# ronghanghu/vit_10b_fsdp_example

Hardware: AMD Instinct MI355X
Metric: images/sec (whole node) for ViT-10B bs=128 224px --fake_data (higher is better)
Workload: dtype bf16; 1 GPU; model=ViT-10B (5120d/32h/32L, patch14, 224px), global_batch=128, seq_len=256, parallelism=fsdp1, grad_ckpt=True, grad_ckpt_blocks=13, fuse_residual=False, init=device

## Files before the change

### csrc/bindings.cpp

```cpp

#include <torch/extension.h>

std::vector<torch::Tensor> layernorm_fwd(torch::Tensor x, torch::Tensor w,
                                         torch::Tensor b, double eps);
std::vector<torch::Tensor> layernorm_bwd(torch::Tensor dy, torch::Tensor x,
                                         torch::Tensor w, torch::Tensor mean,
                                         torch::Tensor rstd);
std::vector<torch::Tensor> layernorm_add_fwd(torch::Tensor x,
                                             torch::Tensor res,
                                             torch::Tensor w, torch::Tensor b,
                                             double eps);
std::vector<torch::Tensor> layernorm_add_bwd(torch::Tensor dy,
                                             torch::Tensor dsum,
                                             torch::Tensor sum,
                                             torch::Tensor w,
                                             torch::Tensor mean,
                                             torch::Tensor rstd);

void fused_adamw(std::vector<torch::Tensor> params,
                 std::vector<torch::Tensor> grads,
                 std::vector<torch::Tensor> exp_avgs,
                 std::vector<torch::Tensor> exp_avg_sqs,
                 std::vector<c10::optional<torch::Tensor>> mirrors,
                 double lr,
                 double beta1, double beta2, double eps, double weight_decay,
                 double bias_c1, double bias_c2,
                 c10::optional<torch::Tensor> grad_scale,
                 double grad_prescale);
torch::Tensor multi_tensor_sqnorm(std::vector<torch::Tensor> tensors);
void multi_tensor_scale(std::vector<torch::Tensor> tensors, double factor);
void multi_tensor_scale_tensor(std::vector<torch::Tensor> tensors,
                               torch::Tensor factor);

std::vector<torch::Tensor> cross_entropy_fwd(torch::Tensor logits,
                                             torch::Tensor target);
torch::Tensor cross_entropy_bwd(torch::Tensor dloss, torch::Tensor logits,
                                torch::Tensor target, torch::Tensor lse);

std::vector<torch::Tensor> fmha_fwd(torch::Tensor q, torch::Tensor k,
                                    torch::Tensor v, double scale,
                                    double p_drop, long seed);
std::vector<torch::Tensor> fmha_bwd(torch::Tensor dout, torch::Tensor q,
                                    torch::Tensor k, torch::Tensor v,
                                    torch::Tensor o, torch::Tensor lse,
                                    double scale, double p_drop, long seed);
std::vector<torch::Tensor> fmha_fwd_qkv(torch::Tensor qkv, long num_heads,
                                        double scale, double p_drop,
                                        long seed);
torch::Tensor fmha_bwd_qkv(torch::Tensor dout, torch::Tensor qkv,
                           torch::Tensor o, torch::Tensor lse,
                           long num_heads, double scale, double p_drop,
                           long seed);
torch::Tensor fmha_rowdot(torch::Tensor dout, torch::Tensor o);
std::vector<torch::Tensor> gelu_bwd_colsum(torch::Tensor dy, torch::Tensor x);
std::vector<torch::Tensor> gelu_bwd_colsum_t(torch::Tensor dy,
                                             torch::Tensor x);
std::vector<torch::Tensor> gelu_dropout_bwd_colsum(torch::Tensor dy,
                                                   torch::Tensor x, double p,
                                                   long seed);
std::vector<torch::Tensor> gelu_dropout_bwd_colsum_t(torch::Tensor dy,
                                                     torch::Tensor x, double p,
                                                     long seed);
torch::Tensor transpose2d(torch::Tensor x);
std::vector<torch::Tensor> transpose_colsum(torch::Tensor x);
torch::Tensor dropout_fwd(torch::Tensor x, double p, long seed);
torch::Tensor dropout_add_fwd(torch::Tensor x, torch::Tensor res, double p,
                              long seed);
torch::Tensor gelu_dropout_fwd(torch::Tensor x, double p, long seed);
torch::Tensor gelu_dropout_bwd(torch::Tensor dy, torch::Tensor x, double p,
                               long seed);
torch::Tensor mfma_probe(torch::Tensor a, torch::Tensor b);
torch::Tensor mfma32_probe(torch::Tensor a, torch::Tensor b);
torch::Tensor tr16_probe(long mode);
std::vector<torch::Tensor> wgrad_gemm(torch::Tensor a, torch::Tensor b,
                                      bool with_bias);
torch::Tensor fwd_gemm(torch::Tensor x, torch::Tensor w,
                       c10::optional<torch::Tensor> bias);
std::vector<torch::Tensor> fwd_gemm_gelu(torch::Tensor x, torch::Tensor w,
                                         torch::Tensor bias);
torch::Tensor lt_gemm(torch::Tensor a, torch::Tensor b, long algo_index,
                      c10::optional<torch::Tensor> bias);
std::vector<torch::Tensor> lt_gemm_gelu(torch::Tensor a, torch::Tensor b,
                                        c10::optional<torch::Tensor> bias,
                                        long algo_index);
std::vector<torch::Tensor> lt_gemm_dgelu_bgrad(torch::Tensor dy,
                                               torch::Tensor w,
                                               torch::Tensor aux,
                                               long algo_index);
torch::Tensor dgrad_tn(torch::Tensor dy, torch::Tensor w, long algo_index);

PYBIND11_MODULE(TORCH_EXTENSION_NAME, m) {
  m.doc() = "MI355X-native CDNA4 kernels for the FSDP ViT framework";
  m.def("layernorm_fwd", &layernorm_fwd, "LayerNorm forward (bf16, fp32 stats)");
  m.def("layernorm_bwd", &layernorm_bwd, "LayerNorm backward");
  m.def("layernorm_add_fwd", &layernorm_add_fwd,
        "fused residual-add + LayerNorm forward");
  m.def("layernorm_add_bwd", &layernorm_add_bwd,
        "fused residual-add + LayerNorm backward");
  m.def("fused_adamw", &fused_adamw,
        "multi-tensor AdamW step (fp32 master, fp32/bf16 grads with "
        "folded prescale + deferred clip)",
        py::arg("params"), py::arg("grads"), py::arg("exp_avgs"),
        py::arg("exp_avg_sqs"), py::arg("mirrors"), py::arg("lr"),
        py::arg("beta1"), py::arg("beta2"), py::arg("eps"),
        py::arg("weight_decay"), py::arg("bias_c1"), py::arg("bias_c2"),
        py::arg("grad_scale") = py::none(), py::arg("grad_prescale") = 1.0);
  m.def("multi_tensor_sqnorm", &multi_tensor_sqnorm,
        "sum of squares over tensor list");
  m.def("multi_tensor_scale", &multi_tensor_scale, "in-place scalar scale");
  m.def("multi_tensor_scale_tensor", &multi_tensor_scale_tensor,
        "in-place scale by device scalar");
  m.def("cross_entropy_fwd", &cross_entropy_fwd, "fused softmax CE forward");
  m.def("cross_entropy_bwd", &cross_entropy_bwd, "fused softmax CE backward");
  m.def("fmha_fwd", &fmha_fwd,
        "flash attention forward (bf16, head_dim<=192; in-kernel "
        "attention dropout via a counter-hash mask)",
        py::arg("q"), py::arg("k"), py::arg("v"), py::arg("scale"),
        py::arg("p_drop") = 0.0, py::arg("seed") = 0);
  m.def("fmha_bwd", &fmha_bwd,
        "flash attention backward (fused FA2-style; regenerates the "
        "dropout mask from the seed)",
        py::arg("dout"), py::arg("q"), py::arg("k"), py::arg("v"),
        py::arg("o"), py::arg("lse"), py::arg("scale"),
        py::arg("p_drop") = 0.0, py::arg("seed") = 0);
  m.def("fmha_fwd_qkv", &fmha_fwd_qkv,
        "flash attention forward on the fused [B,T,3,H,D] qkv projection "
        "(zero-copy strided IO, O returned as [B,T,E])",
        py::arg("qkv"), py::arg("num_heads"), py::arg("scale"),
        py::arg("p_drop") = 0.0, py::arg("seed") = 0);
  m.def("fmha_bwd_qkv", &fmha_bwd_qkv,
        "flash attention backward producing the fused dqkv [B,T,3,H,D]",
        py::arg("dout"), py::arg("qkv"), py::arg("o"), py::arg("lse"),
        py::arg("num_heads"), py::arg("scale"), py::arg("p_drop") = 0.0,
        py::arg("seed") = 0);
  m.def("fmha_rowdot", &fmha_rowdot,
        "Delta = rowsum(dO * O) of the attention backward, fp32 [B,H,T], "
        "for contiguous [B,H,T,D] operands",
        py::arg("dout"), py::arg("o"));
  m.def("gelu_bwd_colsum", &gelu_bwd_colsum,
        "(dx, colsum): exact-erf GELU backward and the bf16 column sums "
        "of dx over all rows (fc1 bias gradient) in one pass",
        py::arg("dy"), py::arg("x"));
  m.def("gelu_bwd_colsum_t", &gelu_bwd_colsum_t,
        "(dx, colsum, dx^T): gelu_bwd_colsum with dx^T [hid, rows] as a "
        "third output; dx and colsum are bit-identical to gelu_bwd_colsum's",
        py::arg("dy"), py::arg("x"));
  m.def("transpose2d", &transpose2d,
        "bf16 [R, C] contiguous -> [C, R] contiguous (C % 8 == 0)",
        py::arg("x"));
  m.def("transpose_colsum", &transpose_colsum,
        "(x^T, colsum): transpose2d plus the bf16 column sums of x over "
        "all rows (a linear's bias gradient) from the same read; fp32 "
        "accumulation in a fixed order",
        py::arg("x"));
  m.def("dropout_fwd", &dropout_fwd,
        "hidden dropout with the in-kernel (seed, row, col) hash mask: "
        "keep ? x / (1 - p) : 0; the same call on dy is its backward",
        py::arg("x"), py::arg("p"), py::arg("seed"));
  m.def("dropout_add_fwd", &dropout_add_fwd,
        "x + dropout(res) in one pass (residual add with the branch's "
        "dropout folded in), rounded once",
        py::arg("x"), py::arg("res"), py::arg("p"), py::arg("seed"));
  m.def("gelu_dropout_fwd", &gelu_dropout_fwd,
        "dropout(gelu(x)) in one pass, exact-erf GELU, rounded once",
        py::arg("x"), py::arg("p"), py::arg("seed"));
  m.def("gelu_dropout_bwd", &gelu_dropout_bwd,
        "backward of gelu_dropout_fwd from dy and the pre-activation x; "
        "regenerates the mask from the seed",
        py::arg("dy"), py::arg("x"), py::arg("p"), py::arg("seed"));
  m.def("gelu_dropout_bwd_colsum", &gelu_dropout_bwd_colsum,
        "(dx, colsum): gelu_dropout_bwd and the bf16 column sums of dx "
        "over all rows (fc1 bias gradient) in one pass; dx is "
        "bit-identical to gelu_dropout_bwd's",
        py::arg("dy"), py::arg("x"), py::arg("p"), py::arg("seed"));
  m.def("gelu_dropout_bwd_colsum_t", &gelu_dropout_bwd_colsum_t,
        "(dx, colsum, dx^T): gelu_dropout_bwd_colsum with dx^T [hid, rows] "
        "as a third output; dx and colsum are bit-identical to "
        "gelu_dropout_bwd_colsum's",
        py::arg("dy"), py::arg("x"), py::arg("p"), py::arg("seed"));
  m.def("mfma_probe", &mfma_probe, "16x16x32 bf16 MFMA layout probe");
  m.def("mfma32_probe", &mfma32_probe, "32x32x16 bf16 MFMA layout probe");
  m.def("tr16_probe", &tr16_probe, "ds_read_b64_tr_b16 semantics probe");
  m.def("wgrad_gemm", &wgrad_gemm,
        "C = A^T B weight-gradient GEMM (bf16, tr16 transpose reads)");
  m.def("fwd_gemm", &fwd_gemm,
        "C = X W^T forward Linear GEMM (+fused bias), hand-written CDNA4 "
        "MFMA (csrc/fgemm.hip)",
        py::arg("x"), py::arg("w"), py::arg("bias") = py::none());
  m.def("fwd_gemm_gelu", &fwd_gemm_gelu,
        "(gelu(X W^T + bias), pre-activation) with the EXACT erf GELU "
        "fused into the hand-written forward GEMM epilogue",
        py::arg("x"), py::arg("w"), py::arg("bias"));
  m.def("lt_gemm", &lt_gemm,
        "row-major bf16 GEMM (+optional fused bias epilogue) via "
        "hipblaslt-ext with an explicit algorithm index (-1 = library "
        "heuristic); offline-search apply path, see "
        "csrc/tools/hipblaslt_search.cpp",
        py::arg("a"), py::arg("b"), py::arg("algo_index") = -1,
        py::arg("bias") = py::none());
  m.def("lt_gemm_gelu", &lt_gemm_gelu,
        "(gelu(a@b+bias), pre-activation aux) in one hipblaslt-ext GEMM "
        "(GELU_AUX epilogue; tanh-approx GELU)",
        py::arg("a"), py::arg("b"), py::arg("bias") = py::none(),
        py::arg("algo_index") = -1);
  m.def("lt_gemm_dgelu_bgrad", &lt_gemm_dgelu_bgrad,
        "(dgelu(dy@w, aux), column-sum bias grad) in one hipblaslt-ext "
        "GEMM (DGELU_BGRAD epilogue)",
        py::arg("dy"), py::arg("w"), py::arg("aux"),
        py::arg("algo_index") = -1);
  m.def("dgrad_tn", &dgrad_tn,
        "dx [tok, in] = dy [tok, out] @ w [out, in] as the library's TN "
        "GEMM on w^T, which csrc/transpose.hip writes into a scratch "
        "buffer on every call; row-contiguous bf16 operands, in and out "
        "multiples of 8, w 16-byte aligned",
        py::arg("dy"), py::arg("w"), py::arg("algo_index") = -1);
}
```

### csrc/fmha.hip

```cpp

#ifndef VITFSDP_KERNELS_ONLY
#include <ATen/cuda/CUDAContext.h>
#include <torch/extension.h>

#include <cstdlib>
#include <cstring>
#include <type_traits>
#endif

#include "mfma_tiles.h"

namespace {

constexpr int kBlockThreads = 256;
constexpr int kKTile = 32;
constexpr int kMaxD = 192;

template <int D>
struct FmhaShapes {
  static constexpr int QSub = (D <= 96) ? 2 : 1;
  static constexpr int QTile = 64 * QSub;
  static constexpr int DP = ((D + 31) / 32) * 32;
  static constexpr int NKC = DP / 32;
  static constexpr int NC = D / 16;
  static constexpr int KStride = DP + 8;
  static constexpr int PStride = kKTile + 8;
  static constexpr int VRow = D + 16;
  struct Shared {
    short k_tile[2][kKTile][KStride];
    short v_tile[2][kKTile][VRow];
  };
  struct SharedDQ {
    short k_tile[kKTile][KStride];
    short v_tile[kKTile][KStride];
  };
  struct SharedDKV {
    short q_tile[32][KStride];
    short do_tile[32][KStride];
    short pt_tile[4][16][PStride];
    short dst_tile[4][16][PStride];
  };
};


struct QkvStrides {
  long qb, qh, qt;
  long ob, oh, ot;
};


template <int D, bool DROP = false>
__global__ __launch_bounds__(kBlockThreads, 3) void fmha_fwd_kernel(
    const short* __restrict__ q, const short* __restrict__ k,
    const short* __restrict__ v, short* __restrict__ o,
    float* __restrict__ lse_out, int T, int H, QkvStrides st, float scale,
    unsigned drop_thresh = 0, float drop_rscale = 1.f, unsigned seed = 0) {
  using S = FmhaShapes<D>;
  constexpr int DP = S::DP, NKC = S::NKC, NC = S::NC;
  constexpr int kQSub = S::QSub;
  constexpr int kQTile = S::QTile;
  HIP_DYNAMIC_SHARED(char, smem_raw)
  typename S::Shared& sm = *reinterpret_cast<typename S::Shared*>(smem_raw);

  const int lane = threadIdx.x & 63;
  const int wave = threadIdx.x >> 6;
  const int col = lane & 15;
  const int seg = lane >> 4;
  const long bh = blockIdx.x;
  const int q_base = blockIdx.y * kQTile;
  const int q_row0 = q_base + wave * (16 * kQSub);

  const int b_idx = (int)(bh / H), h_idx = (int)(bh % H);
  const long qkv_off = (long)b_idx * st.qb + (long)h_idx * st.qh;
  const long o_off = (long)b_idx * st.ob + (long)h_idx * st.oh;

  using KStage = TileStage<kKTile, DP, D, kBlockThreads>;
  using VStage = TileStage<kKTile, D, D, kBlockThreads>;
  const KStage k_stg;
  const VStage v_stg;

  bf16x8 q_frag[kQSub][NKC];
#pragma unroll
  for (int qs = 0; qs < kQSub; ++qs) {
    const int q_row = q_row0 + 16 * qs + col;
    load_row_frags<NKC, D>(q + qkv_off + (long)q_row * st.qt, q_row < T, seg,
                           q_frag[qs]);
  }

  float m_run[kQSub], l_run[kQSub];
  f32x4 o_acc[kQSub][NC];
#pragma unroll
  for (int qs = 0; qs < kQSub; ++qs) {
    m_run[qs] = -INFINITY;
    l_run[qs] = 0.f;
#pragma unroll
    for (int c = 0; c < NC; ++c) o_acc[qs][c] = f32x4{0.f, 0.f, 0.f, 0.f};
  }

  bf16x8 stage[KStage::N > VStage::N ? KStage::N : VStage::N];
  auto issue_k_loads = [&](int k_base) {
    k_stg.load(k + qkv_off, st.qt, k_base, T, stage);
  };
  auto write_k_tile = [&](int buf) { k_stg.store(sm.k_tile[buf], stage); };
  auto issue_v_loads = [&](int k_base) {
    v_stg.load(v + qkv_off, st.qt, k_base, T, stage);
  };
  auto write_v_tile = [&](int buf) { v_stg.store(sm.v_tile[buf], stage); };

  const int n_ktiles = (T + kKTile - 1) / kKTile;
  issue_k_loads(0);
  write_k_tile(0);
  issue_v_loads(0);
  write_v_tile(0);
  __syncthreads();

  int cur = 0;
  for (int kt = 0; kt < n_ktiles; ++kt) {
    const int k_base = kt * kKTile;
    const bool has_next = kt + 1 < n_ktiles;

    if (has_next) issue_k_loads(k_base + kKTile);

#pragma unroll
    for (int qs = 0; qs < kQSub; ++qs) {
      f32x4 st_frag[2] = {{0.f, 0.f, 0.f, 0.f}, {0.f, 0.f, 0.f, 0.f}};
#pragma unroll
      for (int kk = 0; kk < 2; ++kk) {
#pragma unroll
        for (int kc = 0; kc < NKC; ++kc) {
          bf16x8 a_frag = *reinterpret_cast<const bf16x8*>(
              &sm.k_tile[cur][kk * 16 + col][kc * 32 + seg * 8]);
          st_frag[kk] = __builtin_amdgcn_mfma_f32_16x16x32_bf16(
              a_frag, q_frag[qs][kc], st_frag[kk], 0, 0, 0);
        }
      }

      float sc[2][4];
      float my_max = -INFINITY;
#pragma unroll
      for (int kk = 0; kk < 2; ++kk) {
#pragma unroll
        for (int r = 0; r < 4; ++r) {
          float sv = st_frag[kk][r] * scale;
          if (k_base + 16 * kk + seg * 4 + r >= T) sv = -INFINITY;
          sc[kk][r] = sv;
          my_max = fmaxf(my_max, sv);
        }
      }
      my_max = fmaxf(my_max, __shfl_xor(my_max, 16));
      my_max = fmaxf(my_max, __shfl_xor(my_max, 32));
      const float m_new = fmaxf(m_run[qs], my_max);
      const float alpha = __expf(m_run[qs] - m_new);
      m_run[qs] = m_new;

      float p[2][4];
      float row_sum = 0.f;
#pragma unroll
      for (int kk = 0; kk < 2; ++kk) {
#pragma unroll
        for (int r = 0; r < 4; ++r) {
          const float pv =
              (sc[kk][r] == -INFINITY) ? 0.f : __expf(sc[kk][r] - m_new);
          p[kk][r] = pv;
          row_sum += pv;
        }
      }
      row_sum += __shfl_xor(row_sum, 16);
      row_sum += __shfl_xor(row_sum, 32);
      l_run[qs] = l_run[qs] * alpha + row_sum;

      if (DROP) {
        const unsigned qg = (unsigned)(bh * T + q_row0 + 16 * qs + col);
#pragma unroll
        for (int kk = 0; kk < 2; ++kk) {
#pragma unroll
          for (int r = 0; r < 4; ++r) {
            const unsigned kg = (unsigned)(k_base + 16 * kk + seg * 4 + r);
            p[kk][r] = dropout_hash(seed, qg, kg) >= drop_thresh
                           ? p[kk][r] * drop_rscale
                           : 0.f;
          }
        }
      }

      unsigned pk[2][2];
#pragma unroll
      for (int kk = 0; kk < 2; ++kk) {
#pragma unroll
        for (int rr = 0; rr < 2; ++rr)
          pk[kk][rr] = pack_bf16x2(p[kk][2 * rr], p[kk][2 * rr + 1]);
      }
      const bf16x8 pa = c_to_a_layout(pk, seg, col);

#pragma unroll
      for (int r = 0; r < 4; ++r) {
        const float alpha_o = __shfl(alpha, seg * 4 + r);
#pragma unroll
        for (int c = 0; c < NC; ++c) o_acc[qs][c][r] *= alpha_o;
      }

      if (qs == kQSub - 1 && has_next) {
        write_k_tile(cur ^ 1);
        issue_v_loads(k_base + kKTile);
      }

      const unsigned v_lds_base =
          (unsigned)__builtin_amdgcn_groupstaticsize() +
          (unsigned)(offsetof(typename S::Shared, v_tile)) +
          (unsigned)cur * (unsigned)sizeof(sm.v_tile[0]);
      mfma_tr_ring<NC, S::VRow>(pa, v_lds_base, seg, col, o_acc[qs]);
    }

    if (has_next) write_v_tile(cur ^ 1);
    __syncthreads();
    cur ^= 1;
  }

#pragma unroll
  for (int qs = 0; qs < kQSub; ++qs) {
    if (seg == 0) {
      const int q_row = q_row0 + 16 * qs + col;
      if (q_row < T) {
        lse_out[bh * T + q_row] = m_run[qs] + __logf(l_run[qs]);
      }
    }
#pragma unroll
    for (int r = 0; r < 4; ++r) {
      const float l_row = __shfl(l_run[qs], seg * 4 + r);
      const int q_row = q_row0 + 16 * qs + seg * 4 + r;
      if (q_row >= T) continue;
      const float inv_l = (l_row > 0.f) ? 1.f / l_row : 0.f;
      const long out_base = o_off + (long)q_row * st.ot;
#pragma unroll
      for (int c = 0; c < NC; ++c) {
        o[out_base + c * 16 + col] =
            (short)f32_to_bf16(o_acc[qs][c][r] * inv_l);
      }
    }
  }
}

template <int D, bool DROP = false>
__global__ __launch_bounds__(kBlockThreads, 3) void fmha_bwd_dq_kernel(
    const short* __restrict__ q, const short* __restrict__ k,
    const short* __restrict__ v, const short* __restrict__ dout,
    const float* __restrict__ lse, const float* __restrict__ delta,
    short* __restrict__ dq, int T, int H, QkvStrides st, float scale,
    unsigned drop_thresh = 0, float drop_rscale = 1.f, unsigned seed = 0) {
  using S = FmhaShapes<D>;
  constexpr int DP = S::DP, NKC = S::NKC, NC = S::NC;
  constexpr int kQSub = S::QSub;
  constexpr int kQTile = S::QTile;
  HIP_DYNAMIC_SHARED(char, smem_raw)
  typename S::SharedDQ& sm =
      *reinterpret_cast<typename S::SharedDQ*>(smem_raw);

  const int lane = threadIdx.x & 63;
  const int wave = threadIdx.x >> 6;
  const int col = lane & 15;
  const int seg = lane >> 4;
  const long bh = blockIdx.x;
  const int q_base = blockIdx.y * kQTile;
  const int q_row0 = q_base + wave * (16 * kQSub);
  const int b_idx = (int)(bh / H), h_idx = (int)(bh % H);
  const long qkv_off = (long)b_idx * st.qb + (long)h_idx * st.qh;
  const long o_off = (long)b_idx * st.ob + (long)h_idx * st.oh;

  bf16x8 q_frag[kQSub][NKC], do_frag[kQSub][NKC];
  float lse_q[kQSub], delta_q[kQSub];
#pragma unroll
  for (int qs = 0; qs < kQSub; ++qs) {
    const int q_row = q_row0 + 16 * qs + col;
    const bool valid = q_row < T;
    load_row_frags<NKC, D>(q + qkv_off + (long)q_row * st.qt, valid, seg,
                           q_frag[qs]);
    load_row_frags<NKC, D>(dout + o_off + (long)q_row * st.ot, valid, seg,
                           do_frag[qs]);
    lse_q[qs] = valid ? lse[bh * T + q_row] : 0.f;
    delta_q[qs] = valid ? delta[bh * T + q_row] : 0.f;
  }

  f32x4 dq_acc[kQSub][NC];
#pragma unroll
  for (int qs = 0; qs < kQSub; ++qs)
#pragma unroll
    for (int c = 0; c < NC; ++c) dq_acc[qs][c] = f32x4{0.f, 0.f, 0.f, 0.f};

  using Stage = TileStage<kKTile, DP, D, kBlockThreads>;
  const Stage stg;
  bf16x8 kst[Stage::N], vst[Stage::N];
  auto issue_kv_loads = [&](int k_base) {
    stg.load(k + qkv_off, st.qt, k_base, T, kst);
    stg.load(v + qkv_off, st.qt, k_base, T, vst);
  };
  auto write_kv_tiles = [&]() {
    stg.store(sm.k_tile, kst);
    stg.store(sm.v_tile, vst);
  };

  const int n_ktiles = (T + kKTile - 1) / kKTile;
  issue_kv_loads(0);
  write_kv_tiles();
  __syncthreads();
  for (int kt = 0; kt < n_ktiles; ++kt) {
    const int k_base = kt * kKTile;
    const bool has_next = kt + 1 < n_ktiles;
    if (has_next) issue_kv_loads(k_base + kKTile);

#pragma unroll
    for (int qs = 0; qs < kQSub; ++qs) {
      f32x4 st_frag[2] = {{0.f, 0.f, 0.f, 0.f}, {0.f, 0.f, 0.f, 0.f}};
      f32x4 dpt_frag[2] = {{0.f, 0.f, 0.f, 0.f}, {0.f, 0.f, 0.f, 0.f}};
#pragma unroll
      for (int kk = 0; kk < 2; ++kk) {
#pragma unroll
        for (int kc = 0; kc < NKC; ++kc) {
          bf16x8 kb = *reinterpret_cast<const bf16x8*>(
              &sm.k_tile[kk * 16 + col][kc * 32 + seg * 8]);
          bf16x8 vb = *reinterpret_cast<const bf16x8*>(
              &sm.v_tile[kk * 16 + col][kc * 32 + seg * 8]);
          st_frag[kk] = __builtin_amdgcn_mfma_f32_16x16x32_bf16(
              kb, q_frag[qs][kc], st_frag[kk], 0, 0, 0);
          dpt_frag[kk] = __builtin_amdgcn_mfma_f32_16x16x32_bf16(
              vb, do_frag[qs][kc], dpt_frag[kk], 0, 0, 0);
        }
      }

      unsigned pk[2][2];
#pragma unroll
      for (int kk = 0; kk < 2; ++kk) {
#pragma unroll
        for (int rr = 0; rr < 2; ++rr) {
          float ds[2] = {0.f, 0.f};
#pragma unroll
          for (int h = 0; h < 2; ++h) {
            const int r = 2 * rr + h;
            const int k_idx = k_base + 16 * kk + seg * 4 + r;
            if (k_idx < T) {
              const float pv =
                  __expf(st_frag[kk][r] * scale - lse_q[qs]);
              float dp = dpt_frag[kk][r];
              if (DROP) {
                const unsigned qg = (unsigned)(bh * T + q_row0 + 16 * qs + col);
                dp = dropout_hash(seed, qg, (unsigned)k_idx) >= drop_thresh
                         ? dp * drop_rscale
                         : 0.f;
              }
              ds[h] = scale * pv * (dp - delta_q[qs]);
            }
          }
          pk[kk][rr] = pack_bf16x2(ds[0], ds[1]);
        }
      }
      const bf16x8 ds_frag = c_to_a_layout(pk, seg, col);

      const unsigned k_lds_base =
          (unsigned)__builtin_amdgcn_groupstaticsize() +
          (unsigned)offsetof(typename S::SharedDQ, k_tile);
      mfma_tr_ring<NC, S::KStride>(ds_frag, k_lds_base, seg, col,
                                   dq_acc[qs]);
    }

    if (has_next) {
      __syncthreads();
      write_kv_tiles();
      __syncthreads();
    }
  }

#pragma unroll
  for (int qs = 0; qs < kQSub; ++qs) {
#pragma unroll
    for (int r = 0; r < 4; ++r) {
      const int q_row = q_row0 + 16 * qs + seg * 4 + r;
      if (q_row >= T) continue;
      const long out_base = qkv_off + (long)q_row * st.qt;
#pragma unroll
      for (int c = 0; c < NC; ++c) {
        dq[out_base + c * 16 + col] = (short)f32_to_bf16(dq_acc[qs][c][r]);
      }
    }
  }
}

template <int D, bool DROP = false>
__global__ __launch_bounds__(kBlockThreads, 2) void fmha_bwd_dkv_kernel(
    const short* __restrict__ q, const short* __restrict__ k,
    const short* __restrict__ v, const short* __restrict__ dout,
    const float* __restrict__ lse, const float* __restrict__ delta,
    short* __restrict__ dk, short* __restrict__ dv, int T, int H,
    QkvStrides st, float scale,
    unsigned drop_thresh = 0, float drop_rscale = 1.f, unsigned seed = 0) {
  using S = FmhaShapes<D>;
  constexpr int DP = S::DP, NKC = S::NKC, NC = S::NC;
  constexpr int kQStream = 32;
  HIP_DYNAMIC_SHARED(char, smem_raw)
  typename S::SharedDKV& sm =
      *reinterpret_cast<typename S::SharedDKV*>(smem_raw);

  const int lane = threadIdx.x & 63;
  const int wave = threadIdx.x >> 6;
  const int col = lane & 15;
  const int seg = lane >> 4;
  const long bh = blockIdx.x;
  const int k_base = blockIdx.y * 64;
  const int k_row0 = k_base + wave * 16;
  const int b_idx = (int)(bh / H), h_idx = (int)(bh % H);
  const long qkv_off = (long)b_idx * st.qb + (long)h_idx * st.qh;
  const long o_off = (long)b_idx * st.ob + (long)h_idx * st.oh;

  bf16x8 k_frag[NKC], v_frag[NKC];
  {
    const int k_row = k_row0 + col;
    const long base = qkv_off + (long)k_row * st.qt;
    load_row_frags<NKC, D>(k + base, k_row < T, seg, k_frag);
    load_row_frags<NKC, D>(v + base, k_row < T, seg, v_frag);
  }

  f32x4 dk_acc[NC], dv_acc[NC];
#pragma unroll
  for (int c = 0; c < NC; ++c) {
    dk_acc[c] = f32x4{0.f, 0.f, 0.f, 0.f};
    dv_acc[c] = f32x4{0.f, 0.f, 0.f, 0.f};
  }

  using Stage = TileStage<kQStream, DP, D, kBlockThreads>;
  const Stage stg;
  bf16x8 q_st[Stage::N], do_st[Stage::N];
  auto issue_qdo_loads = [&](int q_base) {
    stg.load(q + qkv_off, st.qt, q_base, T, q_st);
    stg.load(dout + o_off, st.ot, q_base, T, do_st);
  };
  auto write_qdo_tiles = [&]() {
    stg.store(sm.q_tile, q_st);
    stg.store(sm.do_tile, do_st);
  };

  const int n_qtiles = (T + kQStream - 1) / kQStream;
  issue_qdo_loads(0);
  write_qdo_tiles();
  __syncthreads();
  for (int qt = 0; qt < n_qtiles; ++qt) {
    const int q_base = qt * kQStream;
    const bool has_next = qt + 1 < n_qtiles;
    if (has_next) issue_qdo_loads(q_base + kQStream);

    f32x4 st_frag[2] = {{0.f, 0.f, 0.f, 0.f}, {0.f, 0.f, 0.f, 0.f}};
    f32x4 dpt_frag[2] = {{0.f, 0.f, 0.f, 0.f}, {0.f, 0.f, 0.f, 0.f}};
#pragma unroll
    for (int qq = 0; qq < 2; ++qq) {
#pragma unroll
      for (int kc = 0; kc < NKC; ++kc) {
        bf16x8 qb = *reinterpret_cast<const bf16x8*>(
            &sm.q_tile[qq * 16 + col][kc * 32 + seg * 8]);
        bf16x8 dob = *reinterpret_cast<const bf16x8*>(
            &sm.do_tile[qq * 16 + col][kc * 32 + seg * 8]);
        st_frag[qq] = __builtin_amdgcn_mfma_f32_16x16x32_bf16(
            k_frag[kc], qb, st_frag[qq], 0, 0, 0);
        dpt_frag[qq] = __builtin_amdgcn_mfma_f32_16x16x32_bf16(
            v_frag[kc], dob, dpt_frag[qq], 0, 0, 0);
      }
    }

#pragma unroll
    for (int qq = 0; qq < 2; ++qq) {
      const int q_idx = q_base + qq * 16 + col;
      const bool q_ok = q_idx < T;
      const float l = q_ok ? lse[bh * T + q_idx] : 0.f;
      const float dlt = q_ok ? delta[bh * T + q_idx] : 0.f;
#pragma unroll
      for (int r = 0; r < 4; ++r) {
        float pt = 0.f, dst = 0.f;
        if (q_ok) {
          pt = __expf(st_frag[qq][r] * scale - l);
          float dp = dpt_frag[qq][r];
          if (DROP) {
            const unsigned qg = (unsigned)(bh * T + q_idx);
            const unsigned kg = (unsigned)(k_row0 + seg * 4 + r);
            const bool keep = dropout_hash(seed, qg, kg) >= drop_thresh;
            dp = keep ? dp * drop_rscale : 0.f;
            dst = scale * pt * (dp - dlt);
            pt = keep ? pt * drop_rscale : 0.f;
          } else {
            dst = scale * pt * (dp - dlt);
          }
        }
        sm.pt_tile[wave][seg * 4 + r][qq * 16 + col] =
            (short)f32_to_bf16(pt);
        sm.dst_tile[wave][seg * 4 + r][qq * 16 + col] =
            (short)f32_to_bf16(dst);
      }
    }
    asm volatile("s_waitcnt lgkmcnt(0)" ::: "memory");

    bf16x8 pt_frag = *reinterpret_cast<const bf16x8*>(
        &sm.pt_tile[wave][col][seg * 8]);
    bf16x8 dst_frag = *reinterpret_cast<const bf16x8*>(
        &sm.dst_tile[wave][col][seg * 8]);
    const unsigned base0 = (unsigned)__builtin_amdgcn_groupstaticsize();
    const unsigned q_lds_base =
        base0 + (unsigned)offsetof(typename S::SharedDKV, q_tile);
    const unsigned do_lds_base =
        base0 + (unsigned)offsetof(typename S::SharedDKV, do_tile);
    mfma_tr_ring<NC, S::KStride>(pt_frag, do_lds_base, seg, col, dv_acc);
    mfma_tr_ring<NC, S::KStride>(dst_frag, q_lds_base, seg, col, dk_acc);
    if (has_next) {
      __syncthreads();
      write_qdo_tiles();
      __syncthreads();
    }
  }

#pragma unroll
  for (int r = 0; r < 4; ++r) {
    const int k_row = k_row0 + seg * 4 + r;
    if (k_row >= T) continue;
    const long out_base = qkv_off + (long)k_row * st.qt;
#pragma unroll
    for (int c = 0; c < NC; ++c) {
      dk[out_base + c * 16 + col] = (short)f32_to_bf16(dk_acc[c][r]);
      dv[out_base + c * 16 + col] = (short)f32_to_bf16(dv_acc[c][r]);
    }
  }
}

constexpr int kRowdotLanes = 8;
constexpr int kRowdotRows = kBlockThreads / kRowdotLanes;
constexpr int kRowdotMaxLoads = kMaxD / 8 / kRowdotLanes;

__global__ __launch_bounds__(kBlockThreads) void fmha_rowdot_kernel(
    const ushort8_t* __restrict__ dout, const ushort8_t* __restrict__ o,
    float* __restrict__ delta, int n_rows, int T, int H, int nvec,
    long sob, long soh, long sot ,
    int h_fast) {
  const int g = threadIdx.x % kRowdotLanes;
  const int slot = threadIdx.x / kRowdotLanes;
  for (long r0 = (long)blockIdx.x * kRowdotRows; r0 < n_rows;
       r0 += (long)gridDim.x * kRowdotRows) {
    const bool ok = r0 + slot < n_rows;
    const unsigned r = ok ? (unsigned)(r0 + slot) : 0u;
    unsigned b, h, t;
    if (h_fast) {
      h = r % (unsigned)H;
      t = (r / (unsigned)H) % (unsigned)T;
    } else {
      t = r % (unsigned)T;
      h = (r / (unsigned)T) % (unsigned)H;
    }
    b = r / ((unsigned)T * (unsigned)H);
    const long base = (long)b * sob + (long)h * soh + (long)t * sot;

    ushort8_t dv[kRowdotMaxLoads], ov[kRowdotMaxLoads];
#pragma unroll
    for (int k = 0; k < kRowdotMaxLoads; ++k) {
      const int v = g + k * kRowdotLanes;
      if (ok && v < nvec) {
        dv[k] = dout[base + v];
        ov[k] = o[base + v];
      }
    }
    float acc[8];
#pragma unroll
    for (int j = 0; j < 8; ++j) acc[j] = 0.f;
#pragma unroll
    for (int k = 0; k < kRowdotMaxLoads; ++k) {
      const int v = g + k * kRowdotLanes;
      if (ok && v < nvec) {
#pragma unroll
        for (int j = 0; j < 8; ++j)
          acc[j] += bf16_to_f32(dv[k][j]) * bf16_to_f32(ov[k][j]);
      }
    }
#pragma unroll
    for (int off = kRowdotLanes / 2; off > 0; off >>= 1) {
#pragma unroll
      for (int j = 0; j < 8; ++j) acc[j] += __shfl_xor(acc[j], off);
    }
#pragma unroll
    for (int j = 0; j < 4; ++j) acc[j] += acc[j + 4];
    acc[0] += acc[2];
    acc[1] += acc[3];
    acc[0] += acc[1];
    if (ok && g == 0) delta[((long)b * H + h) * T + t] = acc[0];
  }
}

__global__ __launch_bounds__(64) void fmha_rowdot_scalar_kernel(
    const unsigned short* __restrict__ dout,
    const unsigned short* __restrict__ o, float* __restrict__ delta, int T,
    int H, int D, long sob, long soh, long sot) {
  const long row = blockIdx.x;
  const int t = (int)(row % T);
  const int h = (int)((row / T) % H);
  const long b = row / ((long)T * H);
  const long base = b * sob + (long)h * soh + (long)t * sot;
  float acc = 0.f;
  for (int i = threadIdx.x; i < D; i += 64)
    acc += bf16_to_f32(dout[base + i]) * bf16_to_f32(o[base + i]);
  acc = wave_all_sum(acc);
  if (threadIdx.x == 0) delta[row] = acc;
}

__global__ __launch_bounds__(256) void fmha_dsoftmax_kernel(
    const unsigned short* __restrict__ s_raw,
    const unsigned short* __restrict__ dp, const float* __restrict__ lse,
    const float* __restrict__ delta, unsigned short* __restrict__ p_out,
    unsigned short* __restrict__ ds_out, int T, float scale) {
  const long row = blockIdx.x;
  const float row_lse = lse[row];
  const float row_delta = delta[row];
  const long base = row * T;
  if ((T & 7) == 0) {
    const int nvec = T / 8;
    const ushort8_t* sv = (const ushort8_t*)(s_raw + base);
    const ushort8_t* dpv = (const ushort8_t*)(dp + base);
    ushort8_t* pv = (ushort8_t*)(p_out + base);
    ushort8_t* dsv = (ushort8_t*)(ds_out + base);
    for (int i = threadIdx.x; i < nvec; i += 256) {
      ushort8_t s8 = sv[i], d8 = dpv[i], p8, ds8;
#pragma unroll
      for (int j = 0; j < 8; ++j) {
        const float p = __expf(bf16_to_f32(s8[j]) * scale - row_lse);
        p8[j] = f32_to_bf16(p);
        ds8[j] = f32_to_bf16(scale * p * (bf16_to_f32(d8[j]) - row_delta));
      }
      pv[i] = p8;
      dsv[i] = ds8;
    }
  } else {
    for (int i = threadIdx.x; i < T; i += 256) {
      const float p = __expf(bf16_to_f32(s_raw[base + i]) * scale - row_lse);
      p_out[base + i] = f32_to_bf16(p);
      ds_out[base + i] =
          f32_to_bf16(scale * p * (bf16_to_f32(dp[base + i]) - row_delta));
    }
  }
}

#ifdef VITFSDP_KERNELS_ONLY
template __global__ void fmha_fwd_kernel<160, false>(
    const short*, const short*, const short*, short*, float*, int, int,
    QkvStrides, float, unsigned, float, unsigned);
template __global__ void fmha_fwd_kernel<160, true>(
    const short*, const short*, const short*, short*, float*, int, int,
    QkvStrides, float, unsigned, float, unsigned);
template __global__ void fmha_fwd_kernel<64, false>(
    const short*, const short*, const short*, short*, float*, int, int,
    QkvStrides, float, unsigned, float, unsigned);
#define VITFSDP_INSTANTIATE_BWD(D_, DROP_)                                  \
  template __global__ void fmha_bwd_dq_kernel<D_, DROP_>(                    \
      const short*, const short*, const short*, const short*, const float*,  \
      const float*, short*, int, int, QkvStrides, float, unsigned, float,    \
      unsigned);                                                             \
  template __global__ void fmha_bwd_dkv_kernel<D_, DROP_>(                   \
      const short*, const short*, const short*, const short*, const float*,  \
      const float*, short*, short*, int, int, QkvStrides, float, unsigned,   \
      float, unsigned);
VITFSDP_INSTANTIATE_BWD(160, false)
VITFSDP_INSTANTIATE_BWD(160, true)
VITFSDP_INSTANTIATE_BWD(64, false)
#undef VITFSDP_INSTANTIATE_BWD
#else
struct FmhaArgs {
  const short *q, *k, *v;
  short* o;
  int B, H, T;
  QkvStrides st;
  float scale;
  float p_drop = 0.f;
  unsigned seed = 0;
};

inline unsigned drop_threshold(float p) {
  if (p <= 0.f) return 0u;
  double t = (double)p * 4294967296.0;
  return t >= 4294967295.0 ? 4294967295u : (unsigned)t;
}

template <typename F>
void with_dropout(const FmhaArgs& a, F&& f) {
  if (a.p_drop > 0.f) {
    f(std::true_type{}, drop_threshold(a.p_drop), 1.f / (1.f - a.p_drop),
      a.seed);
  } else {
    f(std::false_type{}, 0u, 1.f, 0u);
  }
}

template <int D>
void launch_fmha_fwd(const FmhaArgs& a, torch::Tensor& lse) {
  dim3 grid((unsigned)((long)a.B * a.H),
            (a.T + FmhaShapes<D>::QTile - 1) / FmhaShapes<D>::QTile);
  auto stream = at::cuda::getCurrentCUDAStream();
  with_dropout(a, [&](auto drop, unsigned thr, float rs, unsigned seed) {
    hipLaunchKernelGGL((fmha_fwd_kernel<D, decltype(drop)::value>), grid,
                       dim3(kBlockThreads),
                       sizeof(typename FmhaShapes<D>::Shared), stream, a.q,
                       a.k, a.v, a.o, lse.data_ptr<float>(), a.T, a.H, a.st,
                       a.scale, thr, rs, seed);
  });
  HIP_CHECK_LAST();
}

template <int D>
void launch_fmha_bwd(const FmhaArgs& a, const torch::Tensor& lse,
                     const torch::Tensor& delta, short* dq, short* dk,
                     short* dv) {
  using S = FmhaShapes<D>;
  auto stream = at::cuda::getCurrentCUDAStream();
  const unsigned BH = (unsigned)((long)a.B * a.H);
  dim3 grid_dq(BH, (a.T + S::QTile - 1) / S::QTile);
  dim3 grid_dkv(BH, (a.T + 63) / 64);
  with_dropout(a, [&](auto drop, unsigned thr, float rs, unsigned seed) {
    constexpr bool kDrop = decltype(drop)::value;
    hipLaunchKernelGGL((fmha_bwd_dq_kernel<D, kDrop>), grid_dq,
                       dim3(kBlockThreads), sizeof(typename S::SharedDQ),
                       stream, a.q, a.k, a.v, a.o ,
                       lse.data_ptr<float>(), delta.data_ptr<float>(), dq,
                       a.T, a.H, a.st, a.scale, thr, rs, seed);
    HIP_CHECK_LAST();
    hipLaunchKernelGGL((fmha_bwd_dkv_kernel<D, kDrop>), grid_dkv,
                       dim3(kBlockThreads), sizeof(typename S::SharedDKV),
                       stream, a.q, a.k, a.v, a.o ,
                       lse.data_ptr<float>(), delta.data_ptr<float>(), dk, dv,
                       a.T, a.H, a.st, a.scale, thr, rs, seed);
    HIP_CHECK_LAST();
  });
}

#define VITFSDP_FMHA_DISPATCH(D_, expr)                               \
  switch (D_) {                                                       \
    case 16: { constexpr int kD = 16; expr; break; }                  \
    case 32: { constexpr int kD = 32; expr; break; }                  \
    case 48: { constexpr int kD = 48; expr; break; }                  \
    case 64: { constexpr int kD = 64; expr; break; }                  \
    case 80: { constexpr int kD = 80; expr; break; }                  \
    case 96: { constexpr int kD = 96; expr; break; }                  \
    case 112: { constexpr int kD = 112; expr; break; }                \
    case 128: { constexpr int kD = 128; expr; break; }                \
    case 144: { constexpr int kD = 144; expr; break; }                \
    case 160: { constexpr int kD = 160; expr; break; }                \
    case 176: { constexpr int kD = 176; expr; break; }                \
    case 192: { constexpr int kD = 192; expr; break; }                \
    default: TORCH_CHECK(false, "fmha: unsupported head_dim ", D_);   \
  }

#endif

}

#ifndef VITFSDP_KERNELS_ONLY
namespace {

QkvStrides contiguous_strides(int H, int T, int D) {
  QkvStrides st;
  st.qh = (long)T * D;
  st.qb = (long)H * st.qh;
  st.qt = D;
  st.ob = st.qb;
  st.oh = st.qh;
  st.ot = st.qt;
  return st;
}

QkvStrides fused_qkv_strides(int T, int H, int D) {
  QkvStrides st;
  st.qt = 3L * H * D;
  st.qb = (long)T * st.qt;
  st.qh = D;
  st.ot = (long)H * D;
  st.ob = (long)T * st.ot;
  st.oh = D;
  return st;
}

torch::Tensor run_rowdot(const torch::Tensor& dout, const torch::Tensor& o,
                         int B, int H, int T, int D, const QkvStrides& st) {
  auto delta = torch::empty({B, H, T}, dout.options().dtype(torch::kFloat32));
  auto stream = at::cuda::getCurrentCUDAStream();
  const long n_rows = (long)B * H * T;
  if (n_rows == 0) return delta;
  const bool aligned =
      ((reinterpret_cast<uintptr_t>(dout.data_ptr()) |
        reinterpret_cast<uintptr_t>(o.data_ptr())) & 15) == 0 &&
      D % 8 == 0 && D <= kMaxD && st.ob % 8 == 0 && st.oh % 8 == 0 &&
      st.ot % 8 == 0;
  if (aligned && n_rows < (1L << 31)) {
    const long n_blocks =
        std::min<long>((n_rows + kRowdotRows - 1) / kRowdotRows, 2048);
    hipLaunchKernelGGL(fmha_rowdot_kernel, dim3((unsigned)n_blocks),
                       dim3(kBlockThreads), 0, stream,
                       (const ushort8_t*)dout.data_ptr(),
                       (const ushort8_t*)o.data_ptr(), delta.data_ptr<float>(),
                       (int)n_rows, T, H, D / 8, st.ob / 8, st.oh / 8,
                       st.ot / 8, st.oh < st.ot ? 1 : 0);
  } else {
    hipLaunchKernelGGL(fmha_rowdot_scalar_kernel, dim3(n_rows), dim3(64), 0,
                       stream, (const unsigned short*)dout.data_ptr(),
                       (const unsigned short*)o.data_ptr(),
                       delta.data_ptr<float>(), T, H, D, st.ob, st.oh, st.ot);
  }
  HIP_CHECK_LAST();
  return delta;
}

bool supported_head_dim(long D) { return D >= 16 && D <= kMaxD && D % 16 == 0; }

void check_bwd_operand(const char* fn, const char* name,
                       const torch::Tensor& t, const torch::Tensor& like,
                       at::IntArrayRef shape) {
  TORCH_CHECK(t.is_cuda() && t.device() == like.device(), fn, ": ", name,
              " must be a GPU tensor on the device of the other operands");
  TORCH_CHECK(t.scalar_type() == torch::kBFloat16, fn, ": ", name,
              " must be bf16, got ", t.scalar_type());
  TORCH_CHECK(t.sizes() == shape, fn, ": ", name, " must have shape ", shape,
              ", got ", t.sizes());
  TORCH_CHECK(t.is_contiguous(), fn, ": ", name, " must be contiguous");
}

void check_bwd_lse(const char* fn, const torch::Tensor& lse,
                   const torch::Tensor& like, long B, long H, long T) {
  TORCH_CHECK(lse.is_cuda() && lse.device() == like.device(), fn,
              ": lse must be a GPU tensor on the device of the other operands");
  TORCH_CHECK(lse.scalar_type() == torch::kFloat32, fn,
              ": lse must be fp32, got ", lse.scalar_type());
  TORCH_CHECK(lse.dim() == 3 && lse.size(0) == B && lse.size(1) == H &&
                  lse.size(2) == T,
              fn, ": lse must have shape [B, H, T] = [", B, ", ", H, ", ", T,
              "], got ", lse.sizes());
  TORCH_CHECK(lse.is_contiguous(), fn, ": lse must be contiguous");
}

}


std::vector<torch::Tensor> fmha_fwd(torch::Tensor q, torch::Tensor k,
                                    torch::Tensor v, double scale,
                                    double p_drop, long seed) {
  TORCH_CHECK(q.is_cuda() && q.is_contiguous() && k.is_contiguous() &&
              v.is_contiguous());
  TORCH_CHECK(q.scalar_type() == torch::kBFloat16, "fmha_fwd: bf16 only");
  TORCH_CHECK(q.dim() == 4, "fmha_fwd: [B, H, T, D]");
  const int B = q.size(0), H = q.size(1), T = q.size(2), D = q.size(3);
  TORCH_CHECK(D % 16 == 0 && D <= kMaxD,
              "fmha_fwd: head_dim must be a multiple of 16 and <= ", kMaxD);

  auto o = torch::empty_like(q);
  auto lse = torch::empty({B, H, T}, q.options().dtype(torch::kFloat32));
  FmhaArgs a{(const short*)q.data_ptr(), (const short*)k.data_ptr(),
             (const short*)v.data_ptr(), (short*)o.data_ptr(),
             B, H, T, contiguous_strides(H, T, D), (float)scale,
             (float)p_drop, (unsigned)seed};
  VITFSDP_FMHA_DISPATCH(D, launch_fmha_fwd<kD>(a, lse));
  return {o, lse};
}

std::vector<torch::Tensor> fmha_bwd(torch::Tensor dout, torch::Tensor q,
                                    torch::Tensor k, torch::Tensor v,
                                    torch::Tensor o, torch::Tensor lse,
                                    double scale, double p_drop, long seed) {
  TORCH_CHECK(q.is_cuda() && q.dim() == 4,
              "fmha_bwd: q must be a GPU tensor [B, H, T, D]");
  TORCH_CHECK(supported_head_dim(q.size(3)),
              "fmha_bwd: head_dim must be a multiple of 16 and <= ", kMaxD,
              ", got ", q.size(3));
  check_bwd_operand("fmha_bwd", "q", q, q, q.sizes());
  check_bwd_operand("fmha_bwd", "k", k, q, q.sizes());
  check_bwd_operand("fmha_bwd", "v", v, q, q.sizes());
  check_bwd_operand("fmha_bwd", "o", o, q, q.sizes());
  check_bwd_operand("fmha_bwd", "dout", dout, q, q.sizes());
  check_bwd_lse("fmha_bwd", lse, q, q.size(0), q.size(1), q.size(2));
  const int B = q.size(0), H = q.size(1), T = q.size(2), D = q.size(3);
  const QkvStrides st = contiguous_strides(H, T, D);
  auto delta = run_rowdot(dout, o, B, H, T, D, st);
  auto stream = at::cuda::getCurrentCUDAStream();

  static const bool use_compose = [] {
    const char* e = getenv("VITFSDP_FMHA_BWD");
    return e != nullptr && strcmp(e, "compose") == 0;
  }();
  if (use_compose) {
    auto s_raw = at::matmul(q, k.transpose(-2, -1));
    auto dp = at::matmul(dout, v.transpose(-2, -1));
    auto p = torch::empty_like(s_raw);
    auto ds = torch::empty_like(s_raw);
    hipLaunchKernelGGL(fmha_dsoftmax_kernel, dim3((long)B * H * T), dim3(256),
                       0, stream, (const unsigned short*)s_raw.data_ptr(),
                       (const unsigned short*)dp.data_ptr(),
                       lse.data_ptr<float>(), delta.data_ptr<float>(),
                       (unsigned short*)p.data_ptr(),
                       (unsigned short*)ds.data_ptr(), T, (float)scale);
    HIP_CHECK_LAST();
    auto dv = at::matmul(p.transpose(-2, -1), dout);
    auto dq = at::matmul(ds, k);
    auto dk = at::matmul(ds.transpose(-2, -1), q);
    return {dq, dk, dv};
  }

  auto dq = torch::empty_like(q);
  auto dk = torch::empty_like(k);
  auto dv = torch::empty_like(v);
  FmhaArgs a{(const short*)q.data_ptr(), (const short*)k.data_ptr(),
             (const short*)v.data_ptr(), (short*)dout.data_ptr(),
             B, H, T, st, (float)scale, (float)p_drop, (unsigned)seed};
  VITFSDP_FMHA_DISPATCH(
      D, launch_fmha_bwd<kD>(a, lse, delta, (short*)dq.data_ptr(),
                             (short*)dk.data_ptr(), (short*)dv.data_ptr()));
  return {dq, dk, dv};
}

torch::Tensor fmha_rowdot(torch::Tensor dout, torch::Tensor o) {
  TORCH_CHECK(dout.is_cuda() && o.is_cuda() && dout.is_contiguous() &&
                  o.is_contiguous(),
              "fmha_rowdot: contiguous GPU tensors");
  TORCH_CHECK(dout.scalar_type() == torch::kBFloat16 &&
                  o.scalar_type() == torch::kBFloat16,
              "fmha_rowdot: bf16 only");
  TORCH_CHECK(dout.dim() == 4 && dout.sizes() == o.sizes(),
              "fmha_rowdot: two [B, H, T, D] tensors of one shape");
  const int B = dout.size(0), H = dout.size(1), T = dout.size(2),
            D = dout.size(3);
  TORCH_CHECK(D % 16 == 0 && D <= kMaxD,
              "fmha_rowdot: head_dim must be a multiple of 16 and <= ", kMaxD);
  return run_rowdot(dout, o, B, H, T, D, contiguous_strides(H, T, D));
}


std::vector<torch::Tensor> fmha_fwd_qkv(torch::Tensor qkv, long num_heads,
                                        double scale, double p_drop,
                                        long seed) {
  TORCH_CHECK(qkv.is_cuda() && qkv.is_contiguous() && qkv.dim() == 5 &&
                  qkv.size(2) == 3 && qkv.size(3) == num_heads,
              "fmha_fwd_qkv: expected contiguous [B, T, 3, H, D]");
  TORCH_CHECK(qkv.scalar_type() == torch::kBFloat16, "fmha: bf16 only");
  const int B = qkv.size(0), T = qkv.size(1), H = qkv.size(3),
            D = qkv.size(4);
  TORCH_CHECK(D % 16 == 0 && D <= kMaxD,
              "fmha: head_dim must be a multiple of 16 and <= ", kMaxD);
  const QkvStrides st = fused_qkv_strides(T, H, D);

  auto o = torch::empty({B, T, (long)H * D}, qkv.options());
  auto lse = torch::empty({B, H, T}, qkv.options().dtype(torch::kFloat32));
  const short* base = (const short*)qkv.data_ptr();
  FmhaArgs a{base, base + (long)H * D, base + 2L * H * D,
             (short*)o.data_ptr(), B, H, T, st, (float)scale,
             (float)p_drop, (unsigned)seed};
  VITFSDP_FMHA_DISPATCH(D, launch_fmha_fwd<kD>(a, lse));
  return {o, lse};
}

torch::Tensor fmha_bwd_qkv(torch::Tensor dout, torch::Tensor qkv,
                           torch::Tensor o, torch::Tensor lse,
                           long num_heads, double scale, double p_drop,
                           long seed) {
  TORCH_CHECK(qkv.is_cuda() && qkv.is_contiguous() && qkv.dim() == 5 &&
                  qkv.size(2) == 3 && qkv.size(3) == num_heads,
              "fmha_bwd_qkv: expected contiguous GPU qkv [B, T, 3, H, D]");
  TORCH_CHECK(qkv.scalar_type() == torch::kBFloat16,
              "fmha_bwd_qkv: qkv must be bf16, got ", qkv.scalar_type());
  TORCH_CHECK(supported_head_dim(qkv.size(4)),
              "fmha_bwd_qkv: head_dim must be a multiple of 16 and <= ", kMaxD,
              ", got ", qkv.size(4));
  {
    const long b = qkv.size(0), t = qkv.size(1), h = qkv.size(3),
               d = qkv.size(4);
    const std::vector<long> flat{b, t, h * d}, split{b, t, h, d};
    check_bwd_operand("fmha_bwd_qkv", "o", o, qkv,
                      o.dim() == 4 ? split : flat);
    check_bwd_operand("fmha_bwd_qkv", "dout", dout, qkv,
                      dout.dim() == 4 ? split : flat);
    check_bwd_lse("fmha_bwd_qkv", lse, qkv, b, h, t);
  }
  const int B = qkv.size(0), T = qkv.size(1), H = qkv.size(3),
            D = qkv.size(4);
  const QkvStrides st = fused_qkv_strides(T, H, D);
  auto delta = run_rowdot(dout, o, B, H, T, D, st);

  auto dqkv = torch::empty_like(qkv);
  const short* base = (const short*)qkv.data_ptr();
  short* dbase = (short*)dqkv.data_ptr();
  FmhaArgs a{base, base + (long)H * D, base + 2L * H * D,
             (short*)dout.data_ptr(), B, H, T, st, (float)scale,
             (float)p_drop, (unsigned)seed};
  VITFSDP_FMHA_DISPATCH(
      D, launch_fmha_bwd<kD>(a, lse, delta, dbase, dbase + (long)H * D,
                             dbase + 2L * H * D));
  return dqkv;
}
#endif
```

### csrc/mfma_tiles.h

```cpp
#pragma once

#include "common.h"

typedef __attribute__((ext_vector_type(8))) short bf16x8;
typedef __attribute__((ext_vector_type(4))) float f32x4;
typedef __attribute__((ext_vector_type(16))) float f32x16;
typedef __attribute__((ext_vector_type(2))) unsigned int u32x2;


__device__ __forceinline__ u32x2 tr16_read(unsigned lds_byte_addr) {
  u32x2 v;
  asm volatile("ds_read_b64_tr_b16 %0, %1 offset:0"
               : "=v"(v)
               : "v"(lds_byte_addr));
  return v;
}

template <int OFF>
__device__ __forceinline__ u32x2 tr16_read_at(unsigned lds_byte_addr) {
  static_assert(OFF >= 0 && OFF < 65536, "ds offset field is 16 bits");
  u32x2 v;
  asm volatile("ds_read_b64_tr_b16 %0, %1 offset:%2"
               : "=v"(v)
               : "v"(lds_byte_addr), "n"(OFF));
  return v;
}

template <int N>
__device__ __forceinline__ void lds_wait(u32x2& lo, u32x2& hi) {
  asm volatile("s_waitcnt lgkmcnt(%[cnt])"
               : "+v"(lo), "+v"(hi)
               : [cnt] "i"(N)
               : "memory");
}

__device__ __forceinline__ bf16x8 frag_from(u32x2 lo, u32x2 hi) {
  union {
    u32x2 uu[2];
    bf16x8 v;
  } cv;
  cv.uu[0] = lo;
  cv.uu[1] = hi;
  return cv.v;
}

__device__ __forceinline__ unsigned pack_bf16x2(float lo, float hi) {
  return (unsigned)f32_to_bf16(lo) | ((unsigned)f32_to_bf16(hi) << 16);
}

template <int NC, int STRIDE>
__device__ __forceinline__ void mfma_tr_ring(bf16x8 a, unsigned lds_base,
                                             int seg, int col,
                                             f32x4 (&acc)[NC]) {
  const unsigned lane_base =
      lds_base +
      2u * (unsigned)((seg * 8 + (col >> 2)) * STRIDE + (col & 3) * 4);
  u32x2 bf[2][2];
#pragma unroll
  for (int h = 0; h < 2; ++h)
    bf[0][h] = tr16_read(lane_base + 2u * (4 * h * STRIDE));
#pragma unroll
  for (int c = 0; c < NC; ++c) {
    const int cur = c & 1;
    if (c + 1 < NC) {
#pragma unroll
      for (int h = 0; h < 2; ++h)
        bf[cur ^ 1][h] =
            tr16_read(lane_base + 2u * (4 * h * STRIDE + (c + 1) * 16));
      lds_wait<2>(bf[cur][0], bf[cur][1]);
    } else {
      lds_wait<0>(bf[cur][0], bf[cur][1]);
    }
    acc[c] = __builtin_amdgcn_mfma_f32_16x16x32_bf16(
        a, frag_from(bf[cur][0], bf[cur][1]), acc[c], 0, 0, 0);
  }
}

__device__ __forceinline__ bf16x8 c_to_a_layout(const unsigned (&pk)[2][2],
                                                int seg, int col) {
  union {
    unsigned u[4];
    bf16x8 v;
  } cvt;
#pragma unroll
  for (int j2 = 0; j2 < 4; ++j2) {
    const int src = col + 16 * ((seg & 1) * 2 + (j2 >> 1));
    const unsigned lo = (unsigned)__shfl((int)pk[0][j2 & 1], src);
    const unsigned hi = (unsigned)__shfl((int)pk[1][j2 & 1], src);
    cvt.u[j2] = (seg >> 1) ? hi : lo;
  }
  return cvt.v;
}

template <int NKC, int D>
__device__ __forceinline__ void load_row_frags(const short* __restrict__ p,
                                               bool valid, int seg,
                                               bf16x8 (&frag)[NKC]) {
#pragma unroll
  for (int kc = 0; kc < NKC; ++kc) {
    const int d0 = kc * 32 + seg * 8;
    if (valid && d0 + 8 <= D) {
      frag[kc] = *reinterpret_cast<const bf16x8*>(&p[d0]);
    } else {
#pragma unroll
      for (int j = 0; j < 8; ++j)
        frag[kc][j] = (valid && d0 + j < D) ? p[d0 + j] : (short)0;
    }
  }
}

template <int ROWS, int COLS, int D, int THREADS>
struct TileStage {
  static constexpr int VPR = COLS / 8;
  static constexpr int N = (ROWS * VPR + THREADS - 1) / THREADS;
  int r[N], c[N];
  __device__ __forceinline__ TileStage() {
#pragma unroll
    for (int i = 0; i < N; ++i) {
      const int idx = (int)threadIdx.x + i * THREADS;
      r[i] = idx / VPR;
      c[i] = (idx % VPR) * 8;
    }
  }
  template <int M>
  __device__ __forceinline__ void load(const short* __restrict__ p,
                                       long row_stride, int row0, int T,
                                       bf16x8 (&st)[M]) const {
#pragma unroll
    for (int i = 0; i < N; ++i) {
      bf16x8 val = {0, 0, 0, 0, 0, 0, 0, 0};
      const int row = row0 + r[i];
      if (r[i] < ROWS && row < T && (COLS <= D || c[i] < D)) {
        val = *reinterpret_cast<const bf16x8*>(
            &p[(long)row * row_stride + c[i]]);
      }
      st[i] = val;
    }
  }
  template <int STRIDE, int M>
  __device__ __forceinline__ void store(short (*tile)[STRIDE],
                                        const bf16x8 (&st)[M]) const {
#pragma unroll
    for (int i = 0; i < N; ++i) {
      if (r[i] < ROWS) {
        *reinterpret_cast<bf16x8*>(&tile[r[i]][c[i]]) = st[i];
      }
    }
  }
};

__device__ __forceinline__ int xcd_swizzle_m_major(int bid, int nwg) {
  return (bid & 7) * (nwg >> 3) + (bid >> 3);
}

__device__ __forceinline__ void xcd_cluster_tile(int& bx, int& by) {
  bx = blockIdx.x;
  by = blockIdx.y;
  const int gx = gridDim.x, gy = gridDim.y;
  const int nwg = gx * gy;
  const int bid = (int)(blockIdx.x + blockIdx.y * gx);
  int sx = 2, sy = 4;
  if (gy % 4 != 0) {
    if (gy % 2 == 0) { sx = 4; sy = 2; }
    else { sx = 8; sy = 1; }
  }
  if ((nwg & 7) == 0 && gx % sx == 0 && gy % sy == 0) {
    const int xcd = bid & 7, cid = bid >> 3;
    const int lw = gx / sx, lh = gy / sy;
    const int gm = (lw % 4 == 0) ? 4 : ((lw % 2 == 0) ? 2 : 1);
    const int per_band = gm * lh;
    const int band = cid / per_band, r = cid % per_band;
    bx = (xcd % sx) * lw + band * gm + (r % gm);
    by = (xcd / sx) * lh + r / gm;
  } else if ((nwg & 7) == 0) {
    const int swz = xcd_swizzle_m_major(bid, nwg);
    bx = swz % gx;
    by = swz / gx;
  }
}
```

### csrc/probes.hip

```cpp

#ifndef VITFSDP_KERNELS_ONLY
#include <ATen/cuda/CUDAContext.h>
#include <torch/extension.h>
#endif

#include "mfma_tiles.h"

namespace {

__global__ __launch_bounds__(64) void tr16_probe_kernel(
    unsigned short* __restrict__ out, int mode) {
  HIP_DYNAMIC_SHARED(char, smem_raw)
  unsigned short* lds = reinterpret_cast<unsigned short*>(smem_raw);
  for (int i = threadIdx.x; i < 1024; i += 64) lds[i] = (unsigned short)i;
  __syncthreads();
  const int lane = threadIdx.x & 63;
  unsigned addr_elems;
  switch (mode) {
    case 0: addr_elems = 0; break;
    case 1: addr_elems = (lane & 15) + (lane >> 4) * 64; break;
    case 2: addr_elems = (lane & 15) * 4; break;
    default: addr_elems = lane * 4; break;
  }
  unsigned addr = addr_elems * 2 + (unsigned)__builtin_amdgcn_groupstaticsize();
  u32x2 v = tr16_read(addr);
  asm volatile("s_waitcnt lgkmcnt(0)" : "+v"(v) : : "memory");
  out[lane * 4 + 0] = (unsigned short)(v[0] & 0xffff);
  out[lane * 4 + 1] = (unsigned short)(v[0] >> 16);
  out[lane * 4 + 2] = (unsigned short)(v[1] & 0xffff);
  out[lane * 4 + 3] = (unsigned short)(v[1] >> 16);
}

__global__ __launch_bounds__(64) void mfma32_probe_kernel(
    const float* __restrict__ a, const float* __restrict__ b,
    float* __restrict__ c) {
  const int l = threadIdx.x;
  union { unsigned short u[8]; bf16x8 v; } av, bv;
  for (int j = 0; j < 8; ++j) {
    av.u[j] = f32_to_bf16(a[(l & 31) * 16 + (l >> 5) * 8 + j]);
    bv.u[j] = f32_to_bf16(b[((l >> 5) * 8 + j) * 32 + (l & 31)]);
  }
  f32x16 acc = {};
  acc = __builtin_amdgcn_mfma_f32_32x32x16_bf16(av.v, bv.v, acc, 0, 0, 0);
  for (int g = 0; g < 4; ++g)
    for (int r = 0; r < 4; ++r)
      c[((l >> 5) * 4 + g * 8 + r) * 32 + (l & 31)] = acc[g * 4 + r];
}

__global__ __launch_bounds__(64) void mfma_probe_kernel(
    const float* __restrict__ a, const float* __restrict__ b,
    float* __restrict__ c) {
  const int lane = threadIdx.x & 63;
  const int col = lane & 15, seg = lane >> 4;
  bf16x8 af, bf;
#pragma unroll
  for (int j = 0; j < 8; ++j) {
    af[j] = (short)f32_to_bf16(a[col * 32 + seg * 8 + j]);
    bf[j] = (short)f32_to_bf16(b[(seg * 8 + j) * 16 + col]);
  }
  f32x4 acc = {0.f, 0.f, 0.f, 0.f};
  acc = __builtin_amdgcn_mfma_f32_16x16x32_bf16(af, bf, acc, 0, 0, 0);
#pragma unroll
  for (int r = 0; r < 4; ++r) c[(seg * 4 + r) * 16 + col] = acc[r];
}
}

#ifndef VITFSDP_KERNELS_ONLY
torch::Tensor tr16_probe(long mode) {
  auto out = torch::zeros({64, 4}, torch::TensorOptions()
                                       .dtype(torch::kInt16)
                                       .device(torch::kCUDA));
  auto stream = at::cuda::getCurrentCUDAStream();
  hipLaunchKernelGGL(tr16_probe_kernel, dim3(1), dim3(64), 2048, stream,
                     (unsigned short*)out.data_ptr(), (int)mode);
  HIP_CHECK_LAST();
  return out;
}

torch::Tensor mfma32_probe(torch::Tensor a, torch::Tensor b) {
  TORCH_CHECK(a.is_cuda() && a.is_contiguous() && a.dim() == 2 &&
              a.size(0) == 32 && a.size(1) == 16);
  TORCH_CHECK(b.is_cuda() && b.is_contiguous() && b.dim() == 2 &&
              b.size(0) == 16 && b.size(1) == 32);
  TORCH_CHECK(a.scalar_type() == torch::kFloat32 &&
              b.scalar_type() == torch::kFloat32);
  auto c = torch::zeros({32, 32}, a.options());
  auto stream = at::cuda::getCurrentCUDAStream();
  hipLaunchKernelGGL(mfma32_probe_kernel, dim3(1), dim3(64), 0, stream,
                     a.data_ptr<float>(), b.data_ptr<float>(),
                     c.data_ptr<float>());
  HIP_CHECK_LAST();
  return c;
}

torch::Tensor mfma_probe(torch::Tensor a, torch::Tensor b) {
  TORCH_CHECK(a.is_cuda() && a.sizes() == torch::IntArrayRef({16, 32}));
  TORCH_CHECK(b.is_cuda() && b.sizes() == torch::IntArrayRef({32, 16}));
  auto a32 = a.to(torch::kFloat32).contiguous();
  auto b32 = b.to(torch::kFloat32).contiguous();
  auto c = torch::empty({16, 16}, a32.options());
  auto stream = at::cuda::getCurrentCUDAStream();
  hipLaunchKernelGGL(mfma_probe_kernel, dim3(1), dim3(64), 0, stream,
                     a32.data_ptr<float>(), b32.data_ptr<float>(),
                     c.data_ptr<float>());
  HIP_CHECK_LAST();
  return c;
}
#endif
```

Measured before the change: 70.33 images/sec.

## Add 32-row-tile MFMA 32x32x16 flash attention forward and dQ kernels

Adds new flash-attention forward and dQ-backward kernels built on 32x32x16 bf16 MFMA tiles, with 256 query rows per 512-thread block, double-buffered swizzled LDS staging of K/V, and the accumulator reused directly as the next MFMA operand. For head_dim 160/128 these kernels are routed in by default, replacing the 16-row-tile paths, with env/arg overrides. The aim is higher MFMA throughput and fewer LDS round trips in attention. It raises LDS use (large dynamic shared memory) and lowers occupancy, and attention is a small share of ViT-10B step time.

```diff
diff --git a/csrc/bindings.cpp b/csrc/bindings.cpp
--- a/csrc/bindings.cpp
+++ b/csrc/bindings.cpp
@@ -39,18 +39,19 @@
 
 std::vector<torch::Tensor> fmha_fwd(torch::Tensor q, torch::Tensor k,
                                     torch::Tensor v, double scale,
-                                    double p_drop, long seed);
+                                    double p_drop, long seed, long tile);
 std::vector<torch::Tensor> fmha_bwd(torch::Tensor dout, torch::Tensor q,
                                     torch::Tensor k, torch::Tensor v,
                                     torch::Tensor o, torch::Tensor lse,
-                                    double scale, double p_drop, long seed);
+                                    double scale, double p_drop, long seed,
+                                    long tile);
 std::vector<torch::Tensor> fmha_fwd_qkv(torch::Tensor qkv, long num_heads,
                                         double scale, double p_drop,
-                                        long seed);
+                                        long seed, long tile);
 torch::Tensor fmha_bwd_qkv(torch::Tensor dout, torch::Tensor qkv,
                            torch::Tensor o, torch::Tensor lse,
                            long num_heads, double scale, double p_drop,
-                           long seed);
+                           long seed, long tile);
 torch::Tensor fmha_rowdot(torch::Tensor dout, torch::Tensor o);
 std::vector<torch::Tensor> gelu_bwd_colsum(torch::Tensor dy, torch::Tensor x);
 std::vector<torch::Tensor> gelu_bwd_colsum_t(torch::Tensor dy,
@@ -71,6 +72,8 @@
                                long seed);
 torch::Tensor mfma_probe(torch::Tensor a, torch::Tensor b);
 torch::Tensor mfma32_probe(torch::Tensor a, torch::Tensor b);
+torch::Tensor mfma32_acc_operand_probe(torch::Tensor a0, torch::Tensor b0,
+                                       torch::Tensor a_t);
 torch::Tensor tr16_probe(long mode);
 std::vector<torch::Tensor> wgrad_gemm(torch::Tensor a, torch::Tensor b,
                                       bool with_bias);
@@ -116,23 +119,23 @@
         "flash attention forward (bf16, head_dim<=192; in-kernel "
         "attention dropout via a counter-hash mask)",
         py::arg("q"), py::arg("k"), py::arg("v"), py::arg("scale"),
-        py::arg("p_drop") = 0.0, py::arg("seed") = 0);
+        py::arg("p_drop") = 0.0, py::arg("seed") = 0, py::arg("tile") = 0);
   m.def("fmha_bwd", &fmha_bwd,
         "flash attention backward (fused FA2-style; regenerates the "
         "dropout mask from the seed)",
         py::arg("dout"), py::arg("q"), py::arg("k"), py::arg("v"),
         py::arg("o"), py::arg("lse"), py::arg("scale"),
-        py::arg("p_drop") = 0.0, py::arg("seed") = 0);
+        py::arg("p_drop") = 0.0, py::arg("seed") = 0, py::arg("tile") = 0);
   m.def("fmha_fwd_qkv", &fmha_fwd_qkv,
         "flash attention forward on the fused [B,T,3,H,D] qkv projection "
         "(zero-copy strided IO, O returned as [B,T,E])",
         py::arg("qkv"), py::arg("num_heads"), py::arg("scale"),
-        py::arg("p_drop") = 0.0, py::arg("seed") = 0);
+        py::arg("p_drop") = 0.0, py::arg("seed") = 0, py::arg("tile") = 0);
   m.def("fmha_bwd_qkv", &fmha_bwd_qkv,
         "flash attention backward producing the fused dqkv [B,T,3,H,D]",
         py::arg("dout"), py::arg("qkv"), py::arg("o"), py::arg("lse"),
         py::arg("num_heads"), py::arg("scale"), py::arg("p_drop") = 0.0,
-        py::arg("seed") = 0);
+        py::arg("seed") = 0, py::arg("tile") = 0);
   m.def("fmha_rowdot", &fmha_rowdot,
         "Delta = rowsum(dO * O) of the attention backward, fp32 [B,H,T], "
         "for contiguous [B,H,T,D] operands",
@@ -180,6 +183,10 @@
         py::arg("dy"), py::arg("x"), py::arg("p"), py::arg("seed"));
   m.def("mfma_probe", &mfma_probe, "16x16x32 bf16 MFMA layout probe");
   m.def("mfma32_probe", &mfma32_probe, "32x32x16 bf16 MFMA layout probe");
+  m.def("mfma32_acc_operand_probe", &mfma32_acc_operand_probe,
+        "32x32x16 accumulator tile as the next MFMA's B operand, A by "
+        "permuted transposed LDS reads: returns a_t^T (a0 b0)",
+        py::arg("a0"), py::arg("b0"), py::arg("a_t"));
   m.def("tr16_probe", &tr16_probe, "ds_read_b64_tr_b16 semantics probe");
   m.def("wgrad_gemm", &wgrad_gemm,
         "C = A^T B weight-gradient GEMM (bf16, tr16 transpose reads)");
diff --git a/csrc/fmha.hip b/csrc/fmha.hip
--- a/csrc/fmha.hip
+++ b/csrc/fmha.hip
@@ -9,6 +9,7 @@
 #endif
 
 #include "mfma_tiles.h"
+#include "fmha_tile32.h"
 
 namespace {
 
@@ -43,10 +44,6 @@
 };
 
 
-struct QkvStrides {
-  long qb, qh, qt;
-  long ob, oh, ot;
-};
 
 
 template <int D, bool DROP = false>
@@ -660,6 +657,21 @@
 VITFSDP_INSTANTIATE_BWD(160, true)
 VITFSDP_INSTANTIATE_BWD(64, false)
 #undef VITFSDP_INSTANTIATE_BWD
+#define VITFSDP_INSTANTIATE_T32(D_, DROP_)                                  \
+  template __global__ void fmha_fwd_t32_kernel<D_, DROP_>(                   \
+      const short*, const short*, const short*, short*, float*, int, int,    \
+      QkvStrides, float, unsigned, float, unsigned);                         \
+  template __global__ void fmha_bwd_dq_t32_kernel<D_, DROP_>(                \
+      const short*, const short*, const short*, const short*, const float*,  \
+      const float*, short*, int, int, QkvStrides, float, unsigned, float,    \
+      unsigned);
+VITFSDP_INSTANTIATE_T32(160, false)
+VITFSDP_INSTANTIATE_T32(160, true)
+VITFSDP_INSTANTIATE_T32(128, false)
+VITFSDP_INSTANTIATE_T32(128, true)
+VITFSDP_INSTANTIATE_T32(64, false)
+VITFSDP_INSTANTIATE_T32(64, true)
+#undef VITFSDP_INSTANTIATE_T32
 #else
 struct FmhaArgs {
   const short *q, *k, *v;
@@ -688,10 +700,77 @@
 }
 
 template <int D>
-void launch_fmha_fwd(const FmhaArgs& a, torch::Tensor& lse) {
+constexpr bool kHasTile32 = (D == 64 || D == 128 || D == 160);
+
+struct Tile32Route {
+  bool fwd, dq;
+};
+constexpr Tile32Route tile32_default_route(int D, bool drop) {
+  if (D == 160 || D == 128) return {true, true};
+  if (D == 64) return {!drop, false};
+  return {false, false};
+}
+
+inline int fmha_tile_env() {
+  static const int v = [] {
+    const char* e = getenv("VITFSDP_FMHA_TILE");
+    if (e == nullptr || *e == '\0') return 0;
+    const int t = atoi(e);
+    TORCH_CHECK(t == 0 || t == 16 || t == 32,
+                "VITFSDP_FMHA_TILE must be 16 or 32, got ", e);
+    return t;
+  }();
+  return v;
+}
+
+template <int D>
+bool use_tile32(const char* fn, long tile, bool routed) {
+  TORCH_CHECK(tile == 0 || tile == 16 || tile == 32, fn,
+              ": tile must be 0, 16 or 32, got ", tile);
+  if (tile == 32) {
+    TORCH_CHECK(kHasTile32<D>, fn, ": no 32-row-tile kernel for head_dim ", D);
+    return true;
+  }
+  if (tile == 16) return false;
+  const int env = fmha_tile_env();
+  if (env == 16) return false;
+  if (env == 32) return kHasTile32<D>;
+  return kHasTile32<D> && routed;
+}
+
+template <typename Kernel>
+void allow_big_lds(Kernel kernel, size_t bytes) {
+  if (bytes > 64 * 1024) {
+    const hipError_t e = hipFuncSetAttribute(
+        reinterpret_cast<const void*>(kernel),
+        hipFuncAttributeMaxDynamicSharedMemorySize, (int)bytes);
+    TORCH_CHECK(e == hipSuccess, "fmha: cannot reserve ", bytes,
+                " bytes of LDS: ", hipGetErrorString(e));
+  }
+}
+
+template <int D>
+void launch_fmha_fwd(const FmhaArgs& a, torch::Tensor& lse, long tile) {
+  auto stream = at::cuda::getCurrentCUDAStream();
+  if (use_tile32<D>("fmha_fwd", tile, tile32_default_route(D, a.p_drop > 0.f).fwd)) {
+    if constexpr (kHasTile32<D>) {
+      using S32 = Tile32Shapes<D>;
+      dim3 grid32((unsigned)((long)a.B * a.H),
+                  (a.T + kT32QRows - 1) / kT32QRows);
+      with_dropout(a, [&](auto drop, unsigned thr, float rs, unsigned seed) {
+        auto kernel = fmha_fwd_t32_kernel<D, decltype(drop)::value>;
+        allow_big_lds(kernel, sizeof(typename S32::Shared));
+        hipLaunchKernelGGL(kernel, grid32, dim3(kT32Threads),
+                           sizeof(typename S32::Shared), stream, a.q, a.k,
+                           a.v, a.o, lse.data_ptr<float>(), a.T, a.H, a.st,
+                           a.scale, thr, rs, seed);
+      });
+      HIP_CHECK_LAST();
+    }
+    return;
+  }
   dim3 grid((unsigned)((long)a.B * a.H),
             (a.T + FmhaShapes<D>::QTile - 1) / FmhaShapes<D>::QTile);
-  auto stream = at::cuda::getCurrentCUDAStream();
   with_dropout(a, [&](auto drop, unsigned thr, float rs, unsigned seed) {
     hipLaunchKernelGGL((fmha_fwd_kernel<D, decltype(drop)::value>), grid,
                        dim3(kBlockThreads),
@@ -705,19 +784,35 @@
 template <int D>
 void launch_fmha_bwd(const FmhaArgs& a, const torch::Tensor& lse,
                      const torch::Tensor& delta, short* dq, short* dk,
-                     short* dv) {
+                     short* dv, long tile) {
   using S = FmhaShapes<D>;
+  const bool dq32 =
+      use_tile32<D>("fmha_bwd", tile, tile32_default_route(D, a.p_drop > 0.f).dq);
   auto stream = at::cuda::getCurrentCUDAStream();
   const unsigned BH = (unsigned)((long)a.B * a.H);
   dim3 grid_dq(BH, (a.T + S::QTile - 1) / S::QTile);
   dim3 grid_dkv(BH, (a.T + 63) / 64);
   with_dropout(a, [&](auto drop, unsigned thr, float rs, unsigned seed) {
     constexpr bool kDrop = decltype(drop)::value;
-    hipLaunchKernelGGL((fmha_bwd_dq_kernel<D, kDrop>), grid_dq,
-                       dim3(kBlockThreads), sizeof(typename S::SharedDQ),
-                       stream, a.q, a.k, a.v, a.o ,
-                       lse.data_ptr<float>(), delta.data_ptr<float>(), dq,
-                       a.T, a.H, a.st, a.scale, thr, rs, seed);
+    if (dq32) {
+      if constexpr (kHasTile32<D>) {
+        using S32 = Tile32Shapes<D>;
+        auto kernel = fmha_bwd_dq_t32_kernel<D, kDrop>;
+        allow_big_lds(kernel, sizeof(typename S32::Shared));
+        hipLaunchKernelGGL(kernel,
+                           dim3(BH, (a.T + kT32QRows - 1) / kT32QRows),
+                           dim3(kT32Threads), sizeof(typename S32::Shared),
+                           stream, a.q, a.k, a.v, a.o ,
+                           lse.data_ptr<float>(), delta.data_ptr<float>(), dq,
+                           a.T, a.H, a.st, a.scale, thr, rs, seed);
+      }
+    } else {
+      hipLaunchKernelGGL((fmha_bwd_dq_kernel<D, kDrop>), grid_dq,
+                         dim3(kBlockThreads), sizeof(typename S::SharedDQ),
+                         stream, a.q, a.k, a.v, a.o ,
+                         lse.data_ptr<float>(), delta.data_ptr<float>(), dq,
+                         a.T, a.H, a.st, a.scale, thr, rs, seed);
+    }
     HIP_CHECK_LAST();
     hipLaunchKernelGGL((fmha_bwd_dkv_kernel<D, kDrop>), grid_dkv,
                        dim3(kBlockThreads), sizeof(typename S::SharedDKV),
@@ -836,7 +931,7 @@
 
 std::vector<torch::Tensor> fmha_fwd(torch::Tensor q, torch::Tensor k,
                                     torch::Tensor v, double scale,
-                                    double p_drop, long seed) {
+                                    double p_drop, long seed, long tile) {
   TORCH_CHECK(q.is_cuda() && q.is_contiguous() && k.is_contiguous() &&
               v.is_contiguous());
   TORCH_CHECK(q.scalar_type() == torch::kBFloat16, "fmha_fwd: bf16 only");
@@ -851,14 +946,15 @@
              (const short*)v.data_ptr(), (short*)o.data_ptr(),
              B, H, T, contiguous_strides(H, T, D), (float)scale,
              (float)p_drop, (unsigned)seed};
-  VITFSDP_FMHA_DISPATCH(D, launch_fmha_fwd<kD>(a, lse));
+  VITFSDP_FMHA_DISPATCH(D, launch_fmha_fwd<kD>(a, lse, tile));
   return {o, lse};
 }
 
 std::vector<torch::Tensor> fmha_bwd(torch::Tensor dout, torch::Tensor q,
                                     torch::Tensor k, torch::Tensor v,
                                     torch::Tensor o, torch::Tensor lse,
-                                    double scale, double p_drop, long seed) {
+                                    double scale, double p_drop, long seed,
+                                    long tile) {
   TORCH_CHECK(q.is_cuda() && q.dim() == 4,
               "fmha_bwd: q must be a GPU tensor [B, H, T, D]");
   TORCH_CHECK(supported_head_dim(q.size(3)),
@@ -905,7 +1001,8 @@
              B, H, T, st, (float)scale, (float)p_drop, (unsigned)seed};
   VITFSDP_FMHA_DISPATCH(
       D, launch_fmha_bwd<kD>(a, lse, delta, (short*)dq.data_ptr(),
-                             (short*)dk.data_ptr(), (short*)dv.data_ptr()));
+                             (short*)dk.data_ptr(), (short*)dv.data_ptr(),
+                             tile));
   return {dq, dk, dv};
 }
 
@@ -928,7 +1025,7 @@
 
 std::vector<torch::Tensor> fmha_fwd_qkv(torch::Tensor qkv, long num_heads,
                                         double scale, double p_drop,
-                                        long seed) {
+                                        long seed, long tile) {
   TORCH_CHECK(qkv.is_cuda() && qkv.is_contiguous() && qkv.dim() == 5 &&
                   qkv.size(2) == 3 && qkv.size(3) == num_heads,
               "fmha_fwd_qkv: expected contiguous [B, T, 3, H, D]");
@@ -945,14 +1042,14 @@
   FmhaArgs a{base, base + (long)H * D, base + 2L * H * D,
              (short*)o.data_ptr(), B, H, T, st, (float)scale,
              (float)p_drop, (unsigned)seed};
-  VITFSDP_FMHA_DISPATCH(D, launch_fmha_fwd<kD>(a, lse));
+  VITFSDP_FMHA_DISPATCH(D, launch_fmha_fwd<kD>(a, lse, tile));
   return {o, lse};
 }
 
 torch::Tensor fmha_bwd_qkv(torch::Tensor dout, torch::Tensor qkv,
                            torch::Tensor o, torch::Tensor lse,
                            long num_heads, double scale, double p_drop,
-                           long seed) {
+                           long seed, long tile) {
   TORCH_CHECK(qkv.is_cuda() && qkv.is_contiguous() && qkv.dim() == 5 &&
                   qkv.size(2) == 3 && qkv.size(3) == num_heads,
               "fmha_bwd_qkv: expected contiguous GPU qkv [B, T, 3, H, D]");
@@ -984,7 +1081,7 @@
              (float)p_drop, (unsigned)seed};
   VITFSDP_FMHA_DISPATCH(
       D, launch_fmha_bwd<kD>(a, lse, delta, dbase, dbase + (long)H * D,
-                             dbase + 2L * H * D));
+                             dbase + 2L * H * D, tile));
   return dqkv;
 }
 #endif
diff --git a/csrc/fmha_tile32.h b/csrc/fmha_tile32.h
--- /dev/null
+++ b/csrc/fmha_tile32.h
@@ -0,0 +1,438 @@
+#pragma once
+
+#include "mfma_tiles.h"
+
+namespace {
+
+struct QkvStrides {
+  long qb, qh, qt;
+  long ob, oh, ot;
+};
+
+constexpr int kT32Threads = 512;
+constexpr int kT32Waves = 8;
+constexpr int kT32QRows = 32 * kT32Waves;
+constexpr int kT32Keys = 32;
+
+template <int D>
+struct Tile32Shapes {
+  static_assert(D % 32 == 0 && D >= 32 && D <= 192,
+                "32-row tiles need head_dim % 32 == 0");
+  static constexpr int NDS = D / 16;
+  static constexpr int NDB = D / 32;
+  static constexpr int VPR = D / 8;
+  static constexpr int RowChunks = (VPR % 8 == 4) ? VPR : VPR + 4;
+  static constexpr int RowBytes = RowChunks * 16;
+  static constexpr int TileBytes = kT32Keys * RowBytes;
+  static constexpr int kImages = 4;
+  static constexpr int StageBytes = kImages * TileBytes;
+  static constexpr int EpiRowBytes = D * 2 + 16;
+  static constexpr int EpiWaveBytes = 32 * EpiRowBytes;
+  static constexpr int EpiBytes = kT32Waves * EpiWaveBytes;
+  static constexpr int SharedBytes =
+      StageBytes > EpiBytes ? StageBytes : EpiBytes;
+  struct Shared {
+    char bytes[SharedBytes];
+  };
+
+  static constexpr int image_base(int operand, int buf) {
+    return (operand * 2 + buf) * TileBytes;
+  }
+  static constexpr int chunk_off(int row, int ch) {
+    return row * RowBytes + 16 * (ch ^ ((row >> 2) & 3));
+  }
+  static constexpr int row_read_imm(int ds) { return 64 * (ds >> 1); }
+  static constexpr int tr_read_imm(int s, int db) {
+    return s * 16 * RowBytes + db * 64;
+  }
+
+  static_assert(RowChunks % 8 == 4, "bank analysis needs 4 (mod 8) chunks");
+  static_assert(VPR % 4 == 0, "the XOR must stay inside the row's data");
+  static_assert(chunk_off(kT32Keys - 1, VPR - 1) + 16 <= TileBytes &&
+                    chunk_off(kT32Keys - 1, (VPR - 1) ^ 3) + 16 <= TileBytes,
+                "staging store / row read past the image");
+  static_assert(chunk_off(kT32Keys - 1, 3) + row_read_imm(NDS - 1) + 16 <=
+                    TileBytes,
+                "row read past the image");
+  static_assert(chunk_off(15, 3) + 8 + tr_read_imm(1, NDB - 1) + 8 <=
+                    TileBytes,
+                "transposed read past the image");
+  static_assert(image_base(1, 1) + TileBytes <= (int)sizeof(Shared),
+                "images past the shared struct");
+  static_assert((kT32Waves - 1) * EpiWaveBytes + 31 * EpiRowBytes + D * 2 <=
+                    (int)sizeof(Shared),
+                "epilogue rows past the shared struct");
+  static_assert(tr_read_imm(1, NDB - 1) < 65536, "ds offset field");
+};
+
+template <int D>
+struct Tile32Lane {
+  using S = Tile32Shapes<D>;
+  unsigned row_rd[2];
+  unsigned tr_rd[2];
+  __device__ __forceinline__ explicit Tile32Lane(int lane) {
+    const int ql = lane & 31, h = lane >> 5;
+#pragma unroll
+    for (int e = 0; e < 2; ++e)
+      row_rd[e] = (unsigned)(ql * S::RowBytes +
+                             16 * (((e << 1) | h) ^ ((ql >> 2) & 3)));
+#pragma unroll
+    for (int jj = 0; jj < 2; ++jj) {
+      const int row = tr32_lane_row(lane, jj);
+      const int col = tr32_lane_col(lane);
+      tr_rd[jj] = (unsigned)(row * S::RowBytes +
+                             16 * ((col >> 3) ^ ((row >> 2) & 3)) +
+                             2 * (col & 4));
+    }
+  }
+};
+
+template <int D>
+struct Tile32Stage {
+  using S = Tile32Shapes<D>;
+  static constexpr int N = (kT32Keys * S::VPR + kT32Threads - 1) / kT32Threads;
+  int row[N];
+  unsigned lds[N];
+  long gofs[N];
+  __device__ __forceinline__ explicit Tile32Stage(long row_stride) {
+#pragma unroll
+    for (int i = 0; i < N; ++i) {
+      const int idx = (int)threadIdx.x + i * kT32Threads;
+      const int r = idx / S::VPR, ch = idx % S::VPR;
+      row[i] = r;
+      lds[i] = (unsigned)(r * S::RowBytes + 16 * (ch ^ ((r >> 2) & 3)));
+      gofs[i] = (long)r * row_stride + ch * 8;
+    }
+  }
+  __device__ __forceinline__ void load(const short* __restrict__ p,
+                                       long row_stride, int k_base, int T,
+                                       bf16x8 (&st)[N]) const {
+    const short* base = p + (long)k_base * row_stride;
+#pragma unroll
+    for (int i = 0; i < N; ++i) {
+      bf16x8 val = {0, 0, 0, 0, 0, 0, 0, 0};
+      if (row[i] < kT32Keys && k_base + row[i] < T)
+        val = *reinterpret_cast<const bf16x8*>(base + gofs[i]);
+      st[i] = val;
+    }
+  }
+  __device__ __forceinline__ void store(char* image,
+                                        const bf16x8 (&st)[N]) const {
+#pragma unroll
+    for (int i = 0; i < N; ++i) {
+      if (row[i] < kT32Keys)
+        *reinterpret_cast<bf16x8*>(image + lds[i]) = st[i];
+    }
+  }
+};
+
+template <int NDS>
+__device__ __forceinline__ void t32_load_query_frags(
+    const short* __restrict__ row, bool valid, int h, bf16x8 (&frag)[NDS]) {
+#pragma unroll
+  for (int ds = 0; ds < NDS; ++ds) {
+    bf16x8 val = {0, 0, 0, 0, 0, 0, 0, 0};
+    if (valid) val = *reinterpret_cast<const bf16x8*>(&row[16 * ds + 8 * h]);
+    frag[ds] = val;
+  }
+}
+
+template <int D>
+__device__ __forceinline__ void t32_rows_times_query(
+    const char* image, const Tile32Lane<D>& ln,
+    const bf16x8 (&frag)[Tile32Shapes<D>::NDS], f32x16& acc) {
+  using S = Tile32Shapes<D>;
+#pragma unroll
+  for (int ds = 0; ds < S::NDS; ++ds) {
+    const bf16x8 a = *reinterpret_cast<const bf16x8*>(
+        image + ln.row_rd[ds & 1] + S::row_read_imm(ds));
+    acc = __builtin_amdgcn_mfma_f32_32x32x16_bf16(a, frag[ds], acc, 0, 0, 0);
+  }
+}
+
+template <int D, int I>
+struct Tile32TrLoop {
+  using S = Tile32Shapes<D>;
+  static constexpr int NDB = S::NDB;
+  static __device__ __forceinline__ void run(unsigned lo, unsigned hi,
+                                             const bf16x8 (&b)[2],
+                                             f32x16 (&acc)[NDB],
+                                             u32x2 (&ring)[2][2]) {
+    constexpr int cur = I & 1;
+    if constexpr (I + 1 < 2 * NDB) {
+      tr32_read_a<S::tr_read_imm((I + 1) / NDB, (I + 1) % NDB)>(
+          lo, hi, ring[cur ^ 1][0], ring[cur ^ 1][1]);
+      lds_wait<2>(ring[cur][0], ring[cur][1]);
+    } else {
+      lds_wait<0>(ring[cur][0], ring[cur][1]);
+    }
+    acc[I % NDB] = __builtin_amdgcn_mfma_f32_32x32x16_bf16(
+        frag_from(ring[cur][0], ring[cur][1]), b[I / NDB], acc[I % NDB], 0, 0,
+        0);
+    if constexpr (I + 1 < 2 * NDB)
+      Tile32TrLoop<D, I + 1>::run(lo, hi, b, acc, ring);
+  }
+};
+
+template <int D>
+__device__ __forceinline__ void t32_transposed_times_acc(
+    unsigned image_lds, const Tile32Lane<D>& ln, const bf16x8 (&b)[2],
+    f32x16 (&acc)[Tile32Shapes<D>::NDB]) {
+  using S = Tile32Shapes<D>;
+  const unsigned lo = image_lds + ln.tr_rd[0], hi = image_lds + ln.tr_rd[1];
+  u32x2 ring[2][2];
+  tr32_read_a<S::tr_read_imm(0, 0)>(lo, hi, ring[0][0], ring[0][1]);
+  Tile32TrLoop<D, 0>::run(lo, hi, b, acc, ring);
+}
+
+template <int D>
+__device__ __forceinline__ void t32_store_rows(
+    char* smem, int wave, int lane, const f32x16 (&acc)[Tile32Shapes<D>::NDB],
+    float mul, short* __restrict__ dst, long row_stride, int q_row0, int T) {
+  using S = Tile32Shapes<D>;
+  char* region = smem + wave * S::EpiWaveBytes;
+  const int ql = lane & 31, h = lane >> 5;
+#pragma unroll
+  for (int db = 0; db < S::NDB; ++db) {
+#pragma unroll
+    for (int g = 0; g < 4; ++g) {
+      u32x2 w;
+      w[0] = pack_bf16x2(acc[db][4 * g] * mul, acc[db][4 * g + 1] * mul);
+      w[1] = pack_bf16x2(acc[db][4 * g + 2] * mul, acc[db][4 * g + 3] * mul);
+      *reinterpret_cast<u32x2*>(region + ql * S::EpiRowBytes +
+                                2 * (32 * db + 8 * g + 4 * h)) = w;
+    }
+  }
+  __syncthreads();
+  constexpr int kChunks = 32 * S::VPR;
+#pragma unroll
+  for (int it = 0; it < kChunks / 64; ++it) {
+    const int idx = it * 64 + lane;
+    const int r = idx / S::VPR, ch = idx % S::VPR;
+    const bf16x8 val = *reinterpret_cast<const bf16x8*>(
+        region + r * S::EpiRowBytes + ch * 16);
+    if (q_row0 + r < T)
+      *reinterpret_cast<bf16x8*>(dst + (long)(q_row0 + r) * row_stride +
+                                 ch * 8) = val;
+  }
+}
+
+template <int D, bool DROP = false>
+__global__ __launch_bounds__(kT32Threads) void fmha_fwd_t32_kernel(
+    const short* __restrict__ q, const short* __restrict__ k,
+    const short* __restrict__ v, short* __restrict__ o,
+    float* __restrict__ lse_out, int T, int H, QkvStrides st, float scale,
+    unsigned drop_thresh = 0, float drop_rscale = 1.f, unsigned seed = 0) {
+  using S = Tile32Shapes<D>;
+  constexpr int NDS = S::NDS, NDB = S::NDB;
+  HIP_DYNAMIC_SHARED(char, smem)
+  const unsigned smem_lds = (unsigned)__builtin_amdgcn_groupstaticsize();
+
+  const int lane = threadIdx.x & 63;
+  const int wave = threadIdx.x >> 6;
+  const int ql = lane & 31, h = lane >> 5;
+  const long bh = blockIdx.x;
+  const int q_row0 = blockIdx.y * kT32QRows + wave * 32;
+  const int q_row = q_row0 + ql;
+  const int b_idx = (int)(bh / H), h_idx = (int)(bh % H);
+  const long qkv_off = (long)b_idx * st.qb + (long)h_idx * st.qh;
+  const long o_off = (long)b_idx * st.ob + (long)h_idx * st.oh;
+
+  const Tile32Lane<D> ln(lane);
+  const Tile32Stage<D> stg(st.qt);
+
+  bf16x8 qf[NDS];
+  t32_load_query_frags<NDS>(q + qkv_off + (long)q_row * st.qt, q_row < T, h,
+                            qf);
+
+  float m_run = -INFINITY, l_half = 0.f;
+  f32x16 o_acc[NDB];
+#pragma unroll
+  for (int db = 0; db < NDB; ++db)
+#pragma unroll
+    for (int i = 0; i < 16; ++i) o_acc[db][i] = 0.f;
+
+  bf16x8 stage[Tile32Stage<D>::N];
+  const int n_ktiles = (T + kT32Keys - 1) / kT32Keys;
+  stg.load(k + qkv_off, st.qt, 0, T, stage);
+  stg.store(smem + S::image_base(0, 0), stage);
+  stg.load(v + qkv_off, st.qt, 0, T, stage);
+  stg.store(smem + S::image_base(1, 0), stage);
+  __syncthreads();
+
+  int cur = 0;
+  for (int kt = 0; kt < n_ktiles; ++kt) {
+    const int k_base = kt * kT32Keys;
+    const bool has_next = kt + 1 < n_ktiles;
+    if (has_next) stg.load(k + qkv_off, st.qt, k_base + kT32Keys, T, stage);
+
+    f32x16 s_acc;
+#pragma unroll
+    for (int i = 0; i < 16; ++i) s_acc[i] = 0.f;
+    t32_rows_times_query<D>(smem + S::image_base(0, 0) + cur * S::TileBytes,
+                            ln, qf, s_acc);
+
+    float my_max = -INFINITY;
+#pragma unroll
+    for (int i = 0; i < 16; ++i) {
+      float sv = s_acc[i] * scale;
+      if (k_base + 8 * (i >> 2) + 4 * h + (i & 3) >= T) sv = -INFINITY;
+      s_acc[i] = sv;
+      my_max = fmaxf(my_max, sv);
+    }
+    my_max = fmaxf(my_max, __shfl_xor(my_max, 32));
+    const float m_new = fmaxf(m_run, my_max);
+    const float alpha = __expf(m_run - m_new);
+    m_run = m_new;
+
+    float row_sum = 0.f;
+#pragma unroll
+    for (int i = 0; i < 16; ++i) {
+      const float pv =
+          (s_acc[i] == -INFINITY) ? 0.f : __expf(s_acc[i] - m_new);
+      s_acc[i] = pv;
+      row_sum += pv;
+    }
+    l_half = l_half * alpha + row_sum;
+
+    if (DROP) {
+      const unsigned qg = (unsigned)(bh * T + q_row);
+#pragma unroll
+      for (int i = 0; i < 16; ++i) {
+        const unsigned kg =
+            (unsigned)(k_base + 8 * (i >> 2) + 4 * h + (i & 3));
+        s_acc[i] = dropout_hash(seed, qg, kg) >= drop_thresh
+                       ? s_acc[i] * drop_rscale
+                       : 0.f;
+      }
+    }
+    const bf16x8 pf[2] = {acc32_pack_operand<0>(s_acc),
+                          acc32_pack_operand<1>(s_acc)};
+
+#pragma unroll
+    for (int db = 0; db < NDB; ++db) o_acc[db] *= alpha;
+
+    if (has_next) {
+      stg.store(smem + S::image_base(0, 0) + (cur ^ 1) * S::TileBytes, stage);
+      stg.load(v + qkv_off, st.qt, k_base + kT32Keys, T, stage);
+    }
+
+    t32_transposed_times_acc<D>(
+        smem_lds + S::image_base(1, 0) + cur * S::TileBytes, ln, pf, o_acc);
+
+    if (has_next)
+      stg.store(smem + S::image_base(1, 0) + (cur ^ 1) * S::TileBytes, stage);
+    __syncthreads();
+    cur ^= 1;
+  }
+
+  const float l_row = l_half + __shfl_xor(l_half, 32);
+  if (h == 0 && q_row < T) lse_out[bh * T + q_row] = m_run + __logf(l_row);
+  const float inv_l = (l_row > 0.f) ? 1.f / l_row : 0.f;
+  t32_store_rows<D>(smem, wave, lane, o_acc, inv_l, o + o_off, st.ot, q_row0,
+                    T);
+}
+
+template <int D, bool DROP = false>
+__global__ __launch_bounds__(kT32Threads) void fmha_bwd_dq_t32_kernel(
+    const short* __restrict__ q, const short* __restrict__ k,
+    const short* __restrict__ v, const short* __restrict__ dout,
+    const float* __restrict__ lse, const float* __restrict__ delta,
+    short* __restrict__ dq, int T, int H, QkvStrides st, float scale,
+    unsigned drop_thresh = 0, float drop_rscale = 1.f, unsigned seed = 0) {
+  using S = Tile32Shapes<D>;
+  constexpr int NDS = S::NDS, NDB = S::NDB;
+  HIP_DYNAMIC_SHARED(char, smem)
+  const unsigned smem_lds = (unsigned)__builtin_amdgcn_groupstaticsize();
+
+  const int lane = threadIdx.x & 63;
+  const int wave = threadIdx.x >> 6;
+  const int ql = lane & 31, h = lane >> 5;
+  const long bh = blockIdx.x;
+  const int q_row0 = blockIdx.y * kT32QRows + wave * 32;
+  const int q_row = q_row0 + ql;
+  const bool q_ok = q_row < T;
+  const int b_idx = (int)(bh / H), h_idx = (int)(bh % H);
+  const long qkv_off = (long)b_idx * st.qb + (long)h_idx * st.qh;
+  const long o_off = (long)b_idx * st.ob + (long)h_idx * st.oh;
+
+  const Tile32Lane<D> ln(lane);
+  const Tile32Stage<D> stg(st.qt);
+
+  bf16x8 qf[NDS], dof[NDS];
+  t32_load_query_frags<NDS>(q + qkv_off + (long)q_row * st.qt, q_ok, h, qf);
+  t32_load_query_frags<NDS>(dout + o_off + (long)q_row * st.ot, q_ok, h, dof);
+  const float lse_q = q_ok ? lse[bh * T + q_row] : 0.f;
+  const float delta_q = q_ok ? delta[bh * T + q_row] : 0.f;
+
+  f32x16 dq_acc[NDB];
+#pragma unroll
+  for (int db = 0; db < NDB; ++db)
+#pragma unroll
+    for (int i = 0; i < 16; ++i) dq_acc[db][i] = 0.f;
+
+  bf16x8 kst[Tile32Stage<D>::N], vst[Tile32Stage<D>::N];
+  const int n_ktiles = (T + kT32Keys - 1) / kT32Keys;
+  stg.load(k + qkv_off, st.qt, 0, T, kst);
+  stg.load(v + qkv_off, st.qt, 0, T, vst);
+  stg.store(smem + S::image_base(0, 0), kst);
+  stg.store(smem + S::image_base(1, 0), vst);
+  __syncthreads();
+
+  int cur = 0;
+  for (int kt = 0; kt < n_ktiles; ++kt) {
+    const int k_base = kt * kT32Keys;
+    const bool has_next = kt + 1 < n_ktiles;
+
+    f32x16 s_acc, dp_acc;
+#pragma unroll
+    for (int i = 0; i < 16; ++i) {
+      s_acc[i] = 0.f;
+      dp_acc[i] = 0.f;
+    }
+    t32_rows_times_query<D>(smem + S::image_base(0, 0) + cur * S::TileBytes,
+                            ln, qf, s_acc);
+    t32_rows_times_query<D>(smem + S::image_base(1, 0) + cur * S::TileBytes,
+                            ln, dof, dp_acc);
+
+#pragma unroll
+    for (int i = 0; i < 16; ++i) {
+      const int k_idx = k_base + 8 * (i >> 2) + 4 * h + (i & 3);
+      float ds = 0.f;
+      if (k_idx < T) {
+        const float pv = __expf(s_acc[i] * scale - lse_q);
+        float dp = dp_acc[i];
+        if (DROP) {
+          const unsigned qg = (unsigned)(bh * T + q_row);
+          dp = dropout_hash(seed, qg, (unsigned)k_idx) >= drop_thresh
+                   ? dp * drop_rscale
+                   : 0.f;
+        }
+        ds = scale * pv * (dp - delta_q);
+      }
+      s_acc[i] = ds;
+    }
+    const bf16x8 dsf[2] = {acc32_pack_operand<0>(s_acc),
+                           acc32_pack_operand<1>(s_acc)};
+
+    if (has_next) {
+      stg.load(k + qkv_off, st.qt, k_base + kT32Keys, T, kst);
+      stg.load(v + qkv_off, st.qt, k_base + kT32Keys, T, vst);
+    }
+
+    t32_transposed_times_acc<D>(
+        smem_lds + S::image_base(0, 0) + cur * S::TileBytes, ln, dsf, dq_acc);
+
+    if (has_next) {
+      stg.store(smem + S::image_base(0, 0) + (cur ^ 1) * S::TileBytes, kst);
+      stg.store(smem + S::image_base(1, 0) + (cur ^ 1) * S::TileBytes, vst);
+    }
+    __syncthreads();
+    cur ^= 1;
+  }
+
+  t32_store_rows<D>(smem, wave, lane, dq_acc, 1.f, dq + qkv_off, st.qt,
+                    q_row0, T);
+}
+
+}
diff --git a/csrc/mfma_tiles.h b/csrc/mfma_tiles.h
--- a/csrc/mfma_tiles.h
+++ b/csrc/mfma_tiles.h
@@ -74,6 +74,33 @@
     acc[c] = __builtin_amdgcn_mfma_f32_16x16x32_bf16(
         a, frag_from(bf[cur][0], bf[cur][1]), acc[c], 0, 0, 0);
   }
+}
+
+template <int S>
+__device__ __forceinline__ bf16x8 acc32_pack_operand(const f32x16& x) {
+  static_assert(S == 0 || S == 1, "a 32-row tile has two k-steps");
+  union {
+    unsigned u[4];
+    bf16x8 v;
+  } cv;
+#pragma unroll
+  for (int j2 = 0; j2 < 4; ++j2)
+    cv.u[j2] = pack_bf16x2(x[8 * S + 2 * j2], x[8 * S + 2 * j2 + 1]);
+  return cv.v;
+}
+
+__device__ __forceinline__ int tr32_lane_row(int lane, int jj) {
+  return 8 * jj + 4 * (lane >> 5) + ((lane & 15) >> 2);
+}
+__device__ __forceinline__ int tr32_lane_col(int lane) {
+  return 16 * ((lane >> 4) & 1) + 4 * (lane & 3);
+}
+template <int OFF>
+__device__ __forceinline__ void tr32_read_a(unsigned addr_jj0,
+                                            unsigned addr_jj1, u32x2& lo,
+                                            u32x2& hi) {
+  lo = tr16_read_at<OFF>(addr_jj0);
+  hi = tr16_read_at<OFF>(addr_jj1);
 }
 
 __device__ __forceinline__ bf16x8 c_to_a_layout(const unsigned (&pk)[2][2],
diff --git a/csrc/probes.hip b/csrc/probes.hip
--- a/csrc/probes.hip
+++ b/csrc/probes.hip
@@ -47,6 +47,43 @@
       c[((l >> 5) * 4 + g * 8 + r) * 32 + (l & 31)] = acc[g * 4 + r];
 }
 
+__global__ __launch_bounds__(64) void mfma32_acc_operand_probe_kernel(
+    const float* __restrict__ a0, const float* __restrict__ b0,
+    const float* __restrict__ at, float* __restrict__ y) {
+  HIP_DYNAMIC_SHARED(char, smem_raw)
+  unsigned short* lds = reinterpret_cast<unsigned short*>(smem_raw);
+  const int l = threadIdx.x;
+  for (int i = l; i < 32 * 32; i += 64) lds[i] = f32_to_bf16(at[i]);
+  __syncthreads();
+  union { unsigned short u[8]; bf16x8 v; } av, bv;
+  for (int j = 0; j < 8; ++j) {
+    av.u[j] = f32_to_bf16(a0[(l & 31) * 16 + (l >> 5) * 8 + j]);
+    bv.u[j] = f32_to_bf16(b0[((l >> 5) * 8 + j) * 32 + (l & 31)]);
+  }
+  f32x16 x = {};
+  x = __builtin_amdgcn_mfma_f32_32x32x16_bf16(av.v, bv.v, x, 0, 0, 0);
+  const bf16x8 xf[2] = {acc32_pack_operand<0>(x), acc32_pack_operand<1>(x)};
+
+  const unsigned base = (unsigned)__builtin_amdgcn_groupstaticsize();
+  unsigned addr[2];
+  for (int jj = 0; jj < 2; ++jj)
+    addr[jj] =
+        base + 2u * (unsigned)(32 * tr32_lane_row(l, jj) + tr32_lane_col(l));
+  u32x2 lo0, hi0, lo1, hi1;
+  tr32_read_a<0>(addr[0], addr[1], lo0, hi0);
+  tr32_read_a<1024>(addr[0], addr[1], lo1, hi1);
+  lds_wait<2>(lo0, hi0);
+  f32x16 acc = {};
+  acc = __builtin_amdgcn_mfma_f32_32x32x16_bf16(frag_from(lo0, hi0), xf[0],
+                                                acc, 0, 0, 0);
+  lds_wait<0>(lo1, hi1);
+  acc = __builtin_amdgcn_mfma_f32_32x32x16_bf16(frag_from(lo1, hi1), xf[1],
+                                                acc, 0, 0, 0);
+  for (int g = 0; g < 4; ++g)
+    for (int r = 0; r < 4; ++r)
+      y[((l >> 5) * 4 + g * 8 + r) * 32 + (l & 31)] = acc[g * 4 + r];
+}
+
 __global__ __launch_bounds__(64) void mfma_probe_kernel(
     const float* __restrict__ a, const float* __restrict__ b,
     float* __restrict__ c) {
@@ -93,6 +130,25 @@
   return c;
 }
 
+torch::Tensor mfma32_acc_operand_probe(torch::Tensor a0, torch::Tensor b0,
+                                       torch::Tensor a_t) {
+  auto ok = [](const torch::Tensor& t, long r, long c) {
+    return t.is_cuda() && t.is_contiguous() && t.dim() == 2 &&
+           t.size(0) == r && t.size(1) == c &&
+           t.scalar_type() == torch::kFloat32;
+  };
+  TORCH_CHECK(ok(a0, 32, 16) && ok(b0, 16, 32) && ok(a_t, 32, 32),
+              "mfma32_acc_operand_probe: fp32 a0 [32,16], b0 [16,32], "
+              "at [32,32] on the GPU");
+  auto y = torch::zeros({32, 32}, a0.options());
+  auto stream = at::cuda::getCurrentCUDAStream();
+  hipLaunchKernelGGL(mfma32_acc_operand_probe_kernel, dim3(1), dim3(64), 2048,
+                     stream, a0.data_ptr<float>(), b0.data_ptr<float>(),
+                     a_t.data_ptr<float>(), y.data_ptr<float>());
+  HIP_CHECK_LAST();
+  return y;
+}
+
 torch::Tensor mfma_probe(torch::Tensor a, torch::Tensor b) {
   TORCH_CHECK(a.is_cuda() && a.sizes() == torch::IntArrayRef({16, 32}));
   TORCH_CHECK(b.is_cuda() && b.sizes() == torch::IntArrayRef({32, 16}));
```

New measurement: 71.01 images/sec (median of 6 runs). Within noise of the previous version (+1.0%).
